# laertispappas/MPI-k-selection

Measured on AMD Instinct MI355X. Metric: Gkeys/s exact k-th select, 2^30 int32 (1 GPU) / 2^33 (8 GPU); % HBM roofline, higher is better.
Workload: dtype int32; 1 GPU; exact k-th select (median) of 2^30 int32 keys per GPU, uniform_half; n_total=1073741824, k=536870912, keys_per_gpu=1073741824, family=uniform_half, parallelism=single, ranks=1

## Files before the change

include/kth.h:

```cpp
#ifndef KTH_H
#define KTH_H

#include <stddef.h>
#include <stdint.h>

#ifdef __cplusplus
extern "C" {
#endif

#define KTH_OK 0
#define KTH_EINVAL (-1)
#define KTH_ENOMEM (-2)
#define KTH_EHIP (-3)
#define KTH_ENODEV (-4)
#define KTH_EINTERNAL (-5)
#define KTH_ECOMM (-6)

#define KTH_VERSION 1

#define KTH_PATH_LDS 1
#define KTH_PATH_RADIX 2
#define KTH_PATH_WINDOW 3
#define KTH_PATH_WINDOW_FALLBACK 4
#define KTH_PATH_K16 5
#define KTH_PATH_K16_FALLBACK 6

typedef struct kth_ctx kth_ctx;

typedef struct kth_stats {
    int32_t path;
    int32_t mode;
    uint32_t lo_key, hi_key;
    uint64_t n, k;
    uint64_t cnt_lt;
    uint64_t cnt_eq_lo, cnt_eq_hi;
    uint64_t candidates;
    uint64_t capacity;
    int32_t answer;
    int32_t error;
} kth_stats;

const char *kth_strerror(int code);
int kth_version(void);
const char *kth_build_id(void);
int kth_device_count(void);

int kth_select_i32(const int32_t *keys, int64_t n, int64_t k, int32_t *out);

int kth_ctx_create(int device, kth_ctx **ctx);
int kth_ctx_destroy(kth_ctx *ctx);
int kth_ctx_set_stream(kth_ctx *ctx, void *hip_stream);
int kth_ctx_sync(kth_ctx *ctx);
int kth_ctx_reserve(kth_ctx *ctx, int64_t n);

int kth_select_i32_ctx(kth_ctx *ctx, const int32_t *keys, int64_t n, int64_t k, int32_t *out);

int kth_select_i32_async(kth_ctx *ctx, const int32_t *d_keys, int64_t n, int64_t k, int32_t *d_out);

int kth_select_f32(const float *keys, int64_t n, int64_t k, float *out);
int kth_select_f32_ctx(kth_ctx *ctx, const float *keys, int64_t n, int64_t k, float *out);
int kth_select_f32_async(kth_ctx *ctx, const float *d_keys, int64_t n, int64_t k, float *d_out);
uint32_t kth_f32_order_key(float x);
float kth_f32_of_order_key(uint32_t key);

#define KTH_MULTI_MAX_RANKS 8
int kth_select_multi_i32(const int32_t *keys, int64_t n, const int64_t *ks, int m, int32_t *out);
int kth_select_multi_i32_ctx(kth_ctx *ctx, const int32_t *keys, int64_t n, const int64_t *ks, int m, int32_t *out);
int kth_select_multi_i32_async(kth_ctx *ctx, const int32_t *d_keys, int64_t n, const int64_t *ks, int m,
                               int32_t *d_out);
int kth_select_multi_f32(const float *keys, int64_t n, const int64_t *ks, int m, float *out);
int kth_select_multi_f32_ctx(kth_ctx *ctx, const float *keys, int64_t n, const int64_t *ks, int m, float *out);
int kth_select_multi_f32_async(kth_ctx *ctx, const float *d_keys, int64_t n, const int64_t *ks, int m, float *d_out);
int kth_ctx_reserve_multi(kth_ctx *ctx, int64_t n, int m);
int kth_ctx_multi_stats(kth_ctx *ctx, int i, kth_stats *st);

#define KTH_K16_I16  0
#define KTH_K16_U16  1
#define KTH_K16_F16  2
#define KTH_K16_BF16 3
uint16_t kth_k16_order_key(uint16_t bits, int kind);
uint16_t kth_k16_of_order_key(uint16_t key, int kind);
int kth_select_k16(const void *keys, int64_t n, int64_t k, int kind, uint16_t *out);
int kth_select_k16_ctx(kth_ctx *ctx, const void *keys, int64_t n, int64_t k, int kind, uint16_t *out);
int kth_select_k16_async(kth_ctx *ctx, const void *d_keys, int64_t n, int64_t k, int kind, uint16_t *d_out);
int kth_select_multi_k16(const void *keys, int64_t n, const int64_t *ks, int m, int kind, uint16_t *out);
int kth_select_multi_k16_ctx(kth_ctx *ctx, const void *keys, int64_t n, const int64_t *ks, int m, int kind,
                             uint16_t *out);
int kth_select_multi_k16_async(kth_ctx *ctx, const void *d_keys, int64_t n, const int64_t *ks, int m, int kind,
                               uint16_t *d_out);
int kth_ctx_reserve_k16(kth_ctx *ctx, int64_t n, int m);

int kth_ctx_last_stats(kth_ctx *ctx, kth_stats *st);

#define KTH_FINISH_NONE 0
#define KTH_FINISH_COUNTS 1
#define KTH_FINISH_SLICES 2
#define KTH_FINISH_GROUPED 3
#define KTH_FINISH_LEVELS 4
int kth_ctx_last_finish_form(kth_ctx *ctx, int *form);

int kth_ctx_coop(const kth_ctx *ctx);

#define KTH_HOOK_FAULT_TOPK_RANK 1
#define KTH_HOOK_FAULT_BARRIER 2
#define KTH_HOOK_TOPK_SEG_CAP 3
#define KTH_HOOK_K16_MISS 4
#define KTH_HOOK_FINISH_SLICES 5
#define KTH_HOOK_K16_TOPK_NOSKIP 6
int kth_ctx_test_hook(kth_ctx *ctx, int hook, int64_t value);

int kth_ctx_enable_timing(kth_ctx *ctx, int on);
int kth_ctx_take_timing(kth_ctx *ctx, int64_t *n_selects, double *main_ms, double *total_ms);

#define KTH_ROWS_MAX_COLS 16384
int kth_select_rows_i32(kth_ctx *ctx, const int32_t *d_keys, int64_t rows, int32_t cols, int32_t k,
                        int32_t *d_out);
int kth_select_rows_f32(kth_ctx *ctx, const float *d_keys, int64_t rows, int32_t cols, int32_t k,
                        float *d_out);

#define KTH_TOPK_MAX_COLS 4096
int kth_topk_rows_i32(kth_ctx *ctx, const int32_t *d_keys, int64_t rows, int32_t cols, int32_t k, int largest,
                      int32_t *d_vals, int32_t *d_idx);
int kth_topk_rows_f32(kth_ctx *ctx, const float *d_keys, int64_t rows, int32_t cols, int32_t k, int largest,
                      float *d_vals, int32_t *d_idx);

#define KTH_ROWS16_MAX_COLS 8192
int kth_select_rows_k16(kth_ctx *ctx, const void *d_keys, int64_t rows, int32_t cols, int32_t k,
                        int kind, uint16_t *d_out);
int kth_topk_rows_k16(kth_ctx *ctx, const void *d_keys, int64_t rows, int32_t cols, int32_t k, int largest,
                      int kind, uint16_t *d_vals, int32_t *d_idx);

int kth_topk_i32(kth_ctx *ctx, const int32_t *d_keys, int64_t n, int64_t k, int largest, int32_t *d_vals,
                 int64_t *d_idx);
int kth_topk_f32(kth_ctx *ctx, const float *d_keys, int64_t n, int64_t k, int largest, float *d_vals,
                 int64_t *d_idx);

int kth_topk_k16(kth_ctx *ctx, const void *d_keys, int64_t n, int64_t k, int largest, int kind,
                 uint16_t *d_vals, int64_t *d_idx);
int kth_ctx_last_topk_k16_tiles(kth_ctx *ctx, uint64_t *tiles, uint64_t *tiles_read);

#define KTH_WIDE_MAX_COLS   (1 << 24)
#define KTH_WIDE_MAX_SLICES 256
int kth_select_wide_rows_i32(kth_ctx *ctx, const int32_t *d_keys, int64_t rows, int32_t cols, int64_t ld, int32_t k,
                             int32_t *d_out);
int kth_select_wide_rows_f32(kth_ctx *ctx, const float *d_keys, int64_t rows, int32_t cols, int64_t ld, int32_t k,
                             float *d_out);
int kth_topk_wide_rows_i32(kth_ctx *ctx, const int32_t *d_keys, int64_t rows, int32_t cols, int64_t ld, int32_t k,
                           int largest, int32_t *d_vals, int32_t *d_idx);
int kth_topk_wide_rows_f32(kth_ctx *ctx, const float *d_keys, int64_t rows, int32_t cols, int64_t ld, int32_t k,
                           int largest, float *d_vals, int32_t *d_idx);
int kth_ctx_reserve_wide_rows(kth_ctx *ctx, int64_t rows, int32_t cols);
int kth_wide_rows_plan(int64_t rows, int32_t cols, int num_cu, int32_t *slices, int32_t *slice_keys,
                       int32_t *group_rows, int64_t *scratch_bytes);
int kth_ctx_wide_rows_force(kth_ctx *ctx, int32_t slices, int32_t group_rows);

int kth_select_wide_rows_k16(kth_ctx *ctx, const void *d_keys, int64_t rows, int32_t cols, int64_t ld,
                             int32_t k, int kind, uint16_t *d_out);
int kth_topk_wide_rows_k16(kth_ctx *ctx, const void *d_keys, int64_t rows, int32_t cols, int64_t ld,
                           int32_t k, int largest, int kind, uint16_t *d_vals, int32_t *d_idx);
int kth_wide_rows_plan_k16(int64_t rows, int32_t cols, int num_cu, int32_t *slices, int32_t *slice_keys,
                           int32_t *group_rows, int64_t *scratch_bytes);

int kth_select_wide_rows_var_i32(kth_ctx *ctx, const int32_t *d_keys, int64_t rows, int32_t cols, int64_t ld,
                                 const int32_t *d_lens, const int32_t *d_ks, int32_t k, int32_t *d_out);
int kth_select_wide_rows_var_f32(kth_ctx *ctx, const float *d_keys, int64_t rows, int32_t cols, int64_t ld,
                                 const int32_t *d_lens, const int32_t *d_ks, int32_t k, float *d_out);
int kth_select_wide_rows_var_k16(kth_ctx *ctx, const void *d_keys, int64_t rows, int32_t cols, int64_t ld,
                                 const int32_t *d_lens, const int32_t *d_ks, int32_t k, int kind, uint16_t *d_out);
int kth_topk_wide_rows_var_i32(kth_ctx *ctx, const int32_t *d_keys, int64_t rows, int32_t cols, int64_t ld,
                               const int32_t *d_lens, const int32_t *d_ks, int32_t k, int largest, int32_t *d_vals,
                               int32_t *d_idx, int32_t *d_cnt);
int kth_topk_wide_rows_var_f32(kth_ctx *ctx, const float *d_keys, int64_t rows, int32_t cols, int64_t ld,
                               const int32_t *d_lens, const int32_t *d_ks, int32_t k, int largest, float *d_vals,
                               int32_t *d_idx, int32_t *d_cnt);
int kth_topk_wide_rows_var_k16(kth_ctx *ctx, const void *d_keys, int64_t rows, int32_t cols, int64_t ld,
                               const int32_t *d_lens, const int32_t *d_ks, int32_t k, int largest, int kind,
                               uint16_t *d_vals, int32_t *d_idx, int32_t *d_cnt);

int kth_fill_synthetic(kth_ctx *ctx, int32_t *d_out, int64_t n, int64_t offset, int64_t n_total,
                       int dist, uint64_t seed, int32_t param);

int kth_nucleus_wide_rows_f32(kth_ctx *ctx, const float *d_keys, int64_t rows, int32_t cols, int64_t ld,
// ... 59 lines not shown
```

mpi-k-selection_amd/csrc/kth_api.hip:

```cpp
#include <hip/hip_runtime.h>

#include <algorithm>
#include <array>
#include <cmath>
#include <cstdio>
#include <cstdlib>
#include <cstring>
#include <vector>

#include "kth.h"
#include "kth_internal.h"
#include "kth_kernels.hip"
#include "kth_topk.hpp"
#include "kth_k16.hpp"
#include "kth_topk16.hpp"

using kth::SelState;
using kth::StepArgs;
using kth::u64;

namespace {

constexpr int64_t SMALL_N = 16384;
constexpr int64_t RADIX_MAX_N = 1ll << 22;
constexpr int64_t SAMPLE_MAX = 1ll << 20;
constexpr double WINDOW_Z = 5.0;
double window_z() {
    static const double z = [] {
        const char *e = getenv("KTH_WINDOW_Z");
        const double v = e ? atof(e) : 0.0;
        return v > 0.0 ? v : WINDOW_Z;
    }();
    return z;
}
constexpr int LEVEL_GRID_MAX = 1024;
constexpr int POST_DENSE_GRID = 256;
constexpr int64_t HEAD_PER_WG = 16 * 1024;
constexpr int HEAD_GRID_MAX = 64;
static_assert(HEAD_GRID_MAX == SAMPLE_MAX / HEAD_PER_WG, "k_head's grid covers the largest sample");
int gather_grid(u64 nchunks) {
    const u64 per_wg = (u64)(kth::DENSE_BLK / kth::WAVE) * kth::GATHER_BATCH;
    return (int)std::max<u64>(1, (nchunks + per_wg - 1) / per_wg);
}
constexpr size_t ISLOT_WORDS = 3 * (size_t)kth::STATS_WORDS + 2;
constexpr size_t HSLOT_OFF = ISLOT_WORDS;
constexpr size_t HSLOT_WORDS = (size_t)kth::HEAD_LEVELS * kth::STATS_WORDS;
constexpr size_t FSLOT_OFF = HSLOT_OFF + HSLOT_WORDS;
constexpr size_t FSLOT_WORDS = (size_t)kth::FIN_LEVELS * kth::STATS_WORDS;
constexpr size_t PRE_OFF = FSLOT_OFF + FSLOT_WORDS;
static_assert(kth::PRE_WORDS % 4 == 0 && PRE_OFF % 2 == 0, "k_finish clears PreHist in 16-byte words");
constexpr size_t ZERO_WORDS = PRE_OFF + (size_t)kth::PRE_WORDS / 2;
constexpr size_t BAR_OFF = ZERO_WORDS;
constexpr size_t TAIL_OFF = BAR_OFF + kth::BAR_WORDS / 2;
constexpr size_t SLOT_ALLOC_WORDS = TAIL_OFF + kth::FIN_LDS_KEYS / 2;
static_assert(kth::BAR_TAIL % 2 == 0, "the tail word is a u64");
constexpr u64 FIN_SPARSE_PER_WG = (u64)kth::DENSE_BLK * kth::FIN_UNROLL * 4;
constexpr double HEAD_SLACK = 1.5;
static_assert(KTH_STATS_WORDS == kth::STATS_WORDS, "include/kth.h slot size");
constexpr int MAX_EVENTS = 4 * 2048;
constexpr u64 TK_STAGE_MAX_FRAC = 16;
constexpr int TK5_SPLIT = 4;
constexpr int COOP_BACKOFF = 64;
constexpr uint64_t DSCAN_PER_WG = 1ull << 16;
constexpr size_t MSET_HSLOT_OFF = ISLOT_WORDS;
constexpr size_t MSET_WORDS = MSET_HSLOT_OFF + HSLOT_WORDS;
static_assert(KTH_MULTI_MAX_RANKS == kth::MULTI_MAX, "include/kth.h rank limit");
constexpr int MULTI_VARIANTS = 3;
constexpr size_t K16_SHIST_WORDS = kth::K16_VALUES / 2;
constexpr size_t K16_BUF_WORDS = K16_SHIST_WORDS + (size_t)KTH_MULTI_MAX_RANKS * kth::K16_RANK_WORDS;
constexpr size_t K16_HIST_LDS = (size_t)kth::K16_VALUES * 2;
static_assert(KTH_K16_I16 == 0 && KTH_K16_U16 == 1 && KTH_K16_F16 == 2 && KTH_K16_BF16 == 3, "kth_k16.hpp's key kinds");
static_assert(KTH_PATH_K16 == 5 && KTH_PATH_K16_FALLBACK == 6, "kth_k16.hpp's paths");

#define HIP_TRY(x)                                                                                    \
    do {                                                                                              \
        hipError_t e_ = (x);                                                                          \
        if (e_ != hipSuccess) {                                                                       \
            if (getenv("KTH_DEBUG")) fprintf(stderr, "kth: %s failed: %s\n", #x, hipGetErrorString(e_)); \
            return KTH_EHIP;                                                                          \
        }                                                                                             \
    } while (0)

#define KTH_TRY(x)              \
    do {                        \
        int r_ = (x);           \
        if (r_ != KTH_OK) return r_; \
    } while (0)

template <typename T>
struct DevBuf {
    T *p = nullptr;
    u64 count = 0;

    int reserve(u64 want) {
        if (count >= want) return KTH_OK;
        (void)hipDeviceSynchronize();
        release();
        if (hipMalloc(reinterpret_cast<void **>(&p), want * sizeof(T)) != hipSuccess) {
            (void)hipGetLastError();
            p = nullptr;
            return KTH_ENOMEM;
        }
        count = want;
        return KTH_OK;
    }
    void release() {
        if (p) (void)hipFree(p);
        p = nullptr;
        count = 0;
    }
};
template <typename... Bufs>
void release_all(Bufs &...bufs) {
    (bufs.release(), ...);
}

}

struct kth_ctx {
    int device = 0;
    int main_grid[2][7] = {};
    int multi_grid[2][MULTI_VARIANTS] = {};
    int main_wg_per_cu = 0;
    bool fault_topk_rank = false;
    bool fault_barrier = false;
    bool fault_once = false;
    bool topk_stage = true;
    u64 topk_seg_cap = 0;
    u64 sparse_per_wg = 0;
    int post_dense_grid = POST_DENSE_GRID;
    int post_sparse_grid = LEVEL_GRID_MAX;
    bool coop = true;
    bool coop_wanted = true;
    int coop_backoff = 0;
    bool coop_resident = true;
    int fin_grid = 256;
    uint32_t head_slack64 = (uint32_t)(HEAD_SLACK * 64);
    uint32_t head_abs_div = 1024;
    bool pre_hist = true;
    bool group = true;
    bool finish_slices = false;
    hipStream_t stream = nullptr;
    bool own_stream = false;
    int num_cu = 256;
    SelState *st = nullptr;
    u64 *islots = nullptr;
    DevBuf<uint32_t> sample;
    DevBuf<uint32_t> cand;
    DevBuf<uint32_t> gdir;
    DevBuf<uint32_t> cand_rows;
    DevBuf<int32_t> tk_segv;
    DevBuf<uint8_t> tk_segp;
    DevBuf<uint32_t> tk_wcnt;
    DevBuf<uint32_t> tk_wstart;
    kth::TkSeg tk_seg{};
    DevBuf<int32_t> staging;
    DevBuf<u64> topk;
    int32_t *d_status = nullptr;
    int32_t *h_status = nullptr;
    SelState *h_state = nullptr;
    int last_state = -1;
    uint32_t multi_tag = 0;
    DevBuf<SelState> mstate;
    DevBuf<u64> mslots;
    DevBuf<uint32_t> mcand;
    int32_t *d_mstatus = nullptr, *h_mstatus = nullptr;
    int multi_m = 0;
    uint32_t multi_word = 0;
    int multi_set[KTH_MULTI_MAX_RANKS] = {};
    u64 multi_cap = 0;
    bool multi_dirty = false;
    DevBuf<u64> k16;
    DevBuf<kth::K16State> k16st;
    int k16_grid[3] = {};
    bool k16_ready = false;
    bool k16_dirty = false;
    bool k16_miss = false;
    int k16_tf_grid[3] = {};
    u64 tk16_tiles = 0;
    DevBuf<u64> tk16_nread;
    bool k16_topk_noskip = false;
    DevBuf<uint32_t> wide_hist;
    DevBuf<kth::WideState> wide_state;
    DevBuf<uint32_t> wide_cnt;
    bool wide_dirty = false;
    int32_t wide_force_slices = 0, wide_force_group = 0;
    DevBuf<u64> tp_mass;
    DevBuf<uint32_t> tp_cnt;
    DevBuf<kth::TpState> tp_state;
    DevBuf<int32_t> tp_rank;
    bool tp_dirty = false;
    DevBuf<kth::SmState> sm_state;
    DevBuf<uint32_t> sm_loc;
    bool sm_dirty = false;
    bool timing = false;
    std::vector<hipEvent_t> ev_main, ev_total;
    int main_used = 0, total_used = 0;
    bool dirty = false;
    bool count_kept = false;
    bool dist_zero = false;
    bool dist_open = false;
    bool dist_coop_window = false;
    bool counts_left = false;
    u64 *stamps = nullptr;
    int stamp_next = 0;
    u64 *uslots = nullptr;
    int64_t dist_n = 0, dist_k = 0, dist_cap = 0;
    int dist_level_next = 0;
    u64 dscan_per_wg = DSCAN_PER_WG;
    int dist_levels = -1;
    int dist_result_slot = -1;
    int32_t *dist_early_out = nullptr;
    uint32_t *h_dist = nullptr;
    uint32_t *d_dist = nullptr;
    hipEvent_t ev_dist = nullptr;
    uint32_t dist_tag = 0;
};

namespace {

u64 *cand_count(kth_ctx *c) { return c->islots + 3 * (size_t)kth::STATS_WORDS; }

enum : uint32_t { LAST_NONE = 0, LAST_SINGLE = 1, LAST_MULTI = 2, LAST_K16 = 3 };
// ... 178 lines not shown
void over_keys(StepArgs &a, const int32_t *keys, int64_t n) {
    a.keys = keys;
    a.n_local = (u64)n;
}
void over_sample(StepArgs &a, const uint32_t *sample, int64_t s) {
    a.sample = sample;
    a.sample_count = (u64)s;
}
void init_rank(StepArgs &a, int64_t n, int64_t k, int64_t s = 0, u64 r_lo = 0, u64 r_hi = 0) {
    a.init_n = (u64)n;
    a.init_k = (u64)k;
    a.init_s = (u64)s;
    a.r_lo = r_lo;
    a.r_hi = r_hi;
}

void ev_mark(kth_ctx *c, std::vector<hipEvent_t> &pool, int &used) {
    if (!c->timing || used >= (int)pool.size()) return;
    (void)hipEventRecord(pool[used++], c->stream);
}
void ev_main(kth_ctx *c) { ev_mark(c, c->ev_main, c->main_used); }

int launch_check() {
    hipError_t e = hipGetLastError();
    if (e != hipSuccess) {
        if (getenv("KTH_DEBUG")) fprintf(stderr, "kth: launch failed: %s\n", hipGetErrorString(e));
        return KTH_EHIP;
    }
    return KTH_OK;
}

constexpr u64 DENSE_PER_WG = 1ull << 16;
constexpr u64 SPARSE_PER_WG = (u64)kth::BLK * kth::LEVEL_UNROLL * 4;

int level_grid(u64 count, u64 per_wg) {
    u64 g = (count + per_wg - 1) / per_wg;
    return (int)std::max<u64>(1, std::min<u64>(LEVEL_GRID_MAX, g));
}

u64 sparse_wg(const kth_ctx *c) { return c->sparse_per_wg ? c->sparse_per_wg : SPARSE_PER_WG; }

template <bool F32 = false>
void launch_level(kth_ctx *c, StepArgs a, bool dense, int grid) {
    if (dense) {
        a.min_per_wg = DENSE_PER_WG;
        kth::k_level<kth::DENSE_BLK, F32><<<grid, kth::DENSE_BLK, 0, c->stream>>>(a);
    } else {
        a.min_per_wg = sparse_wg(c);
        kth::k_level<kth::BLK, F32><<<grid, kth::BLK, 0, c->stream>>>(a);
    }
}

template <bool F32>
int run_small(kth_ctx *c, const int32_t *keys, int64_t n, int64_t k, int32_t *d_out, int32_t *d_status) {
    c->last_state = 1;
    ev_main(c);
    kth::k_small<F32><<<1, kth::SMALL_BLOCK, (size_t)n * 4, c->stream>>>(keys, (u64)n, (u64)k, d_out, d_status,
                                                                    c->st + 1, d_last(c), single_word<F32>(c, 1));
    ev_main(c);
    return launch_check();
}

kth::CoopArgs coop_args(kth_ctx *c, u64 slot_off, int32_t *d_out, int32_t *d_status) {
    kth::CoopArgs x;
    memset(&x, 0, sizeof x);
    x.slots = c->islots + slot_off;
    x.bar = reinterpret_cast<uint32_t *>(c->islots + BAR_OFF);
    x.tail = reinterpret_cast<uint32_t *>(c->islots + TAIL_OFF);
    x.d_out = d_out;
    x.d_status = d_status;
    x.dense_per_wg = DENSE_PER_WG;
    x.sparse_per_wg = FIN_SPARSE_PER_WG;
    x.slack64 = c->head_slack64;
    x.fault = c->fault_barrier ? 1u : 0u;
    if (c->fault_once) c->fault_barrier = false;
    return x;
}

constexpr size_t FIN_DYN_LDS = (size_t)kth::FIN_LDS_KEYS * 4;
uint32_t *pre_words(kth_ctx *c) { return reinterpret_cast<uint32_t *>(c->islots + PRE_OFF); }

template <bool F32>
void launch_finish(kth_ctx *c, const StepArgs &a, int32_t *d_out, int32_t *d_status, uint32_t last, bool with_pre = false,
                   u64 *head_slots = nullptr, int group_rows = 0) {
    kth::CoopArgs x = coop_args(c, FSLOT_OFF, d_out, d_status);
    x.zero2 = head_slots ? head_slots : c->islots + HSLOT_OFF;
    x.zero2_words = HSLOT_WORDS;
    x.pre = with_pre ? pre_words(c) : nullptr;
    x.last = d_last(c);
    kth::FinGroup fg{nullptr, 0u};
    if (with_pre && group_rows > 0 && !c->finish_slices)
        fg = kth::FinGroup{reinterpret_cast<const uint8_t *>(c->gdir.p), (uint32_t)group_rows};
    kth::k_finish<F32><<<c->fin_grid, kth::DENSE_BLK, FIN_DYN_LDS, c->stream>>>(a, x, last, fg);
}

template <bool F32>
int run_radix(kth_ctx *c, const int32_t *keys, int64_t n, int64_t k, int32_t *d_out, int32_t *d_status) {
    if (c->coop) {
        StepArgs a = Chain{c, c->islots, 3}.next(kth::ADV_INIT_FULL, Chain::NONE);
        over_keys(a, keys, n);
        init_rank(a, n, k);
        ev_main(c);
        launch_finish<F32>(c, a, d_out, d_status, single_word<F32>(c, 1));
        ev_main(c);
        c->last_state = 1;
        return launch_check();
    }
    Chain ch{c, c->islots};
    StepArgs a = ch.next(kth::ADV_INIT_FULL, Chain::ACC | Chain::ZERO);
    over_keys(a, keys, n);
    init_rank(a, n, k);
    ev_main(c);
    launch_level<F32>(c, a, true, level_grid((u64)n, DENSE_PER_WG));
    ev_main(c);
    for (int digit = 1; digit <= 2; ++digit) {
        a = ch.next(kth::ADV_PICK);
        over_keys(a, keys, n);
        launch_level<F32>(c, a, false, level_grid((u64)n, sparse_wg(c)));
    }
    a = ch.next(kth::ADV_PICK, Chain::IN);
    kth::k_result<F32><<<1, kth::BLK, 0, c->stream>>>(a, d_out, d_status, c->islots, ISLOT_WORDS, d_last(c),
                                                     single_word<F32>(c, 1));
    c->last_state = 1;
    return launch_check();
}

StepArgs head_step(Chain &ch, int64_t n, int64_t k, int64_t s, u64 r_lo, u64 r_hi, bool clear_counts) {
    StepArgs a = ch.next(kth::ADV_INIT_SAMPLE, clear_counts ? Chain::ZERO : Chain::NONE);
    if (clear_counts) a.zero_words = 2 * (u64)kth::STATS_WORDS + 1;
    init_rank(a, n, k, s, r_lo, r_hi);
    return a;
}

template <bool F32>
void launch_main(kth_ctx *c, const StepArgs &a, int tflag, uint32_t *tflags, uint32_t *gdir = nullptr) {
    const kth::TkSeg none{};
    if (F32 && tflag >= 5) tflag = 0;
    const int g = c->main_grid[F32][tflag];
    uint32_t *cand = c->cand.p, *rows = c->cand_rows.p;
    switch (tflag) {
    case 1: kth::k_main<1, F32><<<g, kth::BLK, 0, c->stream>>>(a, cand, tflags, nullptr, none); break;
    case 2: kth::k_main<2, F32><<<g, kth::BLK, 0, c->stream>>>(a, cand, tflags, nullptr, none); break;
    case 3: kth::k_main<3, F32><<<g, kth::BLK, 0, c->stream>>>(a, cand, tflags, rows, none); break;
    case 4: kth::k_main<4, F32><<<g, kth::BLK, 0, c->stream>>>(a, cand, tflags, rows, none); break;
    case 5:
        if constexpr (!F32) kth::k_main<5><<<g, kth::BLK, 0, c->stream>>>(a, cand, tflags, nullptr, c->tk_seg);
        break;
    case 6:
        if constexpr (!F32) kth::k_main<6><<<g, kth::BLK, 0, c->stream>>>(a, cand, tflags, nullptr, c->tk_seg);
        break;
    default: kth::k_main<0, F32><<<g, kth::BLK, 0, c->stream>>>(a, cand, gdir, nullptr, none); break;
    }
}

template <bool F32>
int run_window(kth_ctx *c, const int32_t *keys, int64_t n, int64_t k, int32_t *d_out, int32_t *d_status,
               int tflag = 0, uint32_t *tflags = nullptr) {
    const int64_t s = sample_size(n);
    const u64 nchunks = ((u64)s + kth::SAMPLE_CHUNK - 1) / kth::SAMPLE_CHUNK;
    const u64 stride = (u64)n / nchunks;
    u64 r_lo, r_hi;
    window_ranks(n, k, s, &r_lo, &r_hi);
    KTH_TRY(reserve_window(c, n));

    if (c->coop) {
        Chain ch{c, c->islots, 2};
        StepArgs a = head_step(ch, n, k, s, r_lo, r_hi, true);
        kth::CoopArgs hx = coop_args(c, HSLOT_OFF, nullptr, nullptr);
        if (tflag == 0 && c->head_abs_div) hx.abs_min = (u64)s / c->head_abs_div;
        kth::k_head<F32><<<gather_grid(nchunks), kth::DENSE_BLK, 0, c->stream>>>(a, hx, keys, (u64)n, stride,
                                                                               c->sample.p, (u64)s);
        a = ch.next(kth::ADV_CARRY, Chain::ACC);
        over_keys(a, keys, n);
        const bool pre = tflag == 0 && c->pre_hist;
        if (pre) a.pre_hist = pre_words(c);
        const bool grp = pre && grouping(c) && c->gdir.p != nullptr;
        ev_main(c);
        launch_main<F32>(c, a, tflag, tflags, grp ? c->gdir.p : nullptr);
        ev_main(c);
        a = ch.next(kth::ADV_DECIDE, Chain::IN);
        over_keys(a, keys, n);
        launch_finish<F32>(c, a, d_out, d_status, single_word<F32>(c, 0), pre, nullptr, grp ? c->main_grid[F32][0] : 0);
        c->last_state = 0;
        c->counts_left = true;
        return launch_check();
    }
    Chain ch{c, c->islots};
    StepArgs a = ch.next(kth::ADV_INIT_SAMPLE, Chain::ACC | Chain::ZERO);
    init_rank(a, n, k, s, r_lo, r_hi);
    kth::k_gather<true, F32><<<gather_grid(nchunks), kth::DENSE_BLK, 0, c->stream>>>(a, keys, (u64)n, stride,
                                                                                   c->sample.p, (u64)s);
    const int gs = level_grid((u64)s, sparse_wg(c));
    for (int digit = 2; digit <= 3; ++digit) {
        a = ch.next(kth::ADV_PICK);
        over_sample(a, c->sample.p, s);
        launch_level(c, a, false, gs);
    }
    a = ch.next(kth::ADV_PICK);
    over_keys(a, keys, n);
    ev_main(c);
    launch_main<F32>(c, a, tflag, tflags);
    ev_main(c);
    a = ch.next(kth::ADV_DECIDE);
    over_keys(a, keys, n);
    launch_level<F32>(c, a, true, c->post_dense_grid);
    for (int digit = 2; digit <= 3; ++digit) {
        a = ch.next(kth::ADV_PICK);
        over_keys(a, keys, n);
        launch_level<F32>(c, a, false, c->post_sparse_grid);
    }
    a = ch.next(kth::ADV_PICK, Chain::IN);
    const bool keep_count = tflag == 3 || tflag == 4;
    kth::k_result<F32><<<1, kth::BLK, 0, c->stream>>>(a, d_out, d_status, c->islots,
                                                     keep_count ? 3 * (u64)kth::STATS_WORDS : (u64)ISLOT_WORDS,
                                                     d_last(c), single_word<F32>(c, 1));
    if (keep_count) c->count_kept = true;
    c->last_state = 1;
    return launch_check();
}

void coop_tick(kth_ctx *c) {
    if (c->coop_backoff > 0 && --c->coop_backoff == 0) c->coop = c->coop_wanted;
}

template <bool F32 = false>
int select_enqueue(kth_ctx *c, const int32_t *d_keys, int64_t n, int64_t k, int32_t *d_out, int32_t *d_status,
                   int tflag = 0, uint32_t *tflags = nullptr) {
    if (c->dirty || c->count_kept) {
        HIP_TRY(hipMemsetAsync(c->islots, 0, SLOT_ALLOC_WORDS * sizeof(u64), c->stream));
        c->dirty = c->count_kept = false;
    }
    int rc;
    ev_mark(c, c->ev_total, c->total_used);
    if (n <= SMALL_N)
        rc = run_small<F32>(c, d_keys, n, k, d_out, d_status);
    else if (n <= RADIX_MAX_N)
        rc = run_radix<F32>(c, d_keys, n, k, d_out, d_status);
    else
        rc = run_window<F32>(c, d_keys, n, k, d_out, d_status, tflag, tflags);
    ev_mark(c, c->ev_total, c->total_used);
    if (rc != KTH_OK) c->dirty = true;
    if (c->stamps) dump_stamps(c);
    return rc;
}

template <bool F32 = false>
int select_async(kth_ctx *c, const int32_t *d_keys, int64_t n, int64_t k, int32_t *d_out, int32_t *d_status,
                 int tflag = 0, uint32_t *tflags = nullptr) {
    if (!c || !d_keys || (!d_out && !d_status) || n < 1 || k < 1 || k > n) return KTH_EINVAL;
    KTH_TRY(set_device(c));
    coop_tick(c);
    return select_enqueue<F32>(c, d_keys, n, k, d_out, d_status, tflag, tflags);
}

bool is_device_ptr(const void *p) {
    hipPointerAttribute_t at;
    hipError_t e = hipPointerGetAttributes(&at, p);
    if (e != hipSuccess) {
        (void)hipGetLastError();
        return false;
    }
    return at.type == hipMemoryTypeDevice || at.type == hipMemoryTypeManaged;
}

thread_local kth_ctx *tl_ctx = nullptr;
// ... 438 lines not shown
        HIP_TRY(hipMemsetAsync(c->sm_state.p, 0, c->sm_state.count * sizeof(kth::SmState), c->stream));
    c->sm_dirty = false;
    return KTH_OK;
}

template <class K, bool VEC>
int launch_sample_group(kth_ctx *c, const WidePlan &p, const typename K::elem *keys, int64_t g, uint32_t cols, u64 ld,
                        const kth::TopP &v, bool no_a, const float *us, int32_t *d_tok, int32_t *d_cnt) {
    if (p.slices == 1) {
        kth::k_sm_fused<K, VEC><<<(int)g, kth::WD_FBLOCK, 0, c->stream>>>(keys, ld, cols, v, us, d_tok, d_cnt);
        return launch_check();
    }
    const dim3 grid((unsigned)p.slices, (unsigned)g);
    const uint32_t sk = (uint32_t)p.slice_keys;
    kth::k_sm_max<K, VEC><<<grid, kth::WD_BLOCK, 0, c->stream>>>(keys, ld, cols, sk, c->sm_state.p, v);
    for (int phase = no_a ? 1 : 0; phase < 2; ++phase)
        for (int pass = 0; pass < K::PASSES; ++pass) {
            kth::k_sm_count<K, VEC><<<grid, kth::WD_BLOCK, 0, c->stream>>>(keys, ld, cols, sk, phase, pass, c->tp_mass.p,
                                                                        c->tp_cnt.p, c->sm_state.p, v);
            kth::k_sm_pick<K><<<(int)g, kth::WD_BLOCK, 0, c->stream>>>(c->tp_mass.p, c->tp_cnt.p, c->sm_state.p, phase, pass,
                                                                     cols, v, us);
        }
    kth::k_sm_loc_count<K, VEC><<<grid, kth::WD_BLOCK, 0, c->stream>>>(keys, ld, cols, sk, c->sm_state.p, c->sm_loc.p, v);
    kth::k_sm_loc_pick<K, VEC><<<grid, kth::WD_BLOCK, 0, c->stream>>>(keys, ld, cols, sk, c->sm_state.p, c->sm_loc.p, v,
                                                                   d_tok, d_cnt);
    const int rc = launch_check();
    if (rc != KTH_OK) c->tp_dirty = c->sm_dirty = true;
    return rc;
}

template <class K>
int sample_rows(kth_ctx *c, const typename K::elem *keys, int64_t rows, int32_t cols, int64_t ld, const kth::TopP &var,
                bool no_a, const float *d_us, int32_t *d_tok, int32_t *d_cnt) {
    constexpr int32_t align = K::PER;
    WidePlan p = wide_plan(rows, cols, c->num_cu, c->wide_force_slices, c->wide_force_group, align,
                           align == 8 ? WIDE16_MIN_SLICE : WIDE_MIN_SLICE);
    if (p.slices > 1) {
        p.group_rows = (int32_t)std::min<int64_t>(p.group_rows, SM_GROUP_MAX);
        KTH_TRY(reserve_sample(c, p.group_rows));
    }
    const bool vec = (reinterpret_cast<uintptr_t>(keys) & 15u) == 0 && ld % align == 0;
    const auto launch = vec ? launch_sample_group<K, true> : launch_sample_group<K, false>;
    for (int64_t r0 = 0; r0 < rows; r0 += p.group_rows) {
        const int64_t g = std::min<int64_t>(p.group_rows, rows - r0);
        kth::TopP v = var;
        if (v.lens) v.lens += r0;
        if (v.ps) v.ps += r0;
        if (v.temps) v.temps += r0;
        if (v.ks) v.ks += r0;
        KTH_TRY(launch(c, p, keys + (u64)r0 * (u64)ld, g, (uint32_t)cols, (u64)ld, v, no_a, d_us + r0, d_tok + r0,
                       d_cnt ? d_cnt + r0 : nullptr));
    }
    return KTH_OK;
}

int sample_entry(kth_ctx *c, const void *d_keys, int64_t rows, int32_t cols, int64_t ld, const int32_t *d_lens,
                 const int32_t *d_ks, int32_t k, const float *d_ps, float p, const float *d_temps, float temp,
                 const float *d_us, int kind, int32_t *d_tok, int32_t *d_cnt) {
    if (!c || !d_keys || !d_us || !d_tok || rows < 0 || cols < 1 || cols > KTH_WIDE_MAX_COLS || ld < cols)
        return KTH_EINVAL;
    if (kind != -1 && kind != KTH_K16_F16 && kind != KTH_K16_BF16) return KTH_EINVAL;
    if (!(temp > 0.0f) || !std::isfinite(temp) || (!d_ps && std::isnan(p))) return KTH_EINVAL;
    if (rows == 0) return KTH_OK;
    KTH_TRY(set_device(c));
    const kth::TopP var{d_lens, d_ps, d_temps, d_ks, p, temp, k};
    const bool no_a = !d_ps && p >= 1.0f && !d_ks && k <= 0;
    if (kind == -1)
        return sample_rows<kth::TpF32>(c, static_cast<const uint32_t *>(d_keys), rows, cols, ld, var, no_a, d_us, d_tok,
                                       d_cnt);
    const uint16_t *keys = static_cast<const uint16_t *>(d_keys);
    if (kind == KTH_K16_BF16) return sample_rows<kth::TpK16<true>>(c, keys, rows, cols, ld, var, no_a, d_us, d_tok, d_cnt);
    return sample_rows<kth::TpK16<false>>(c, keys, rows, cols, ld, var, no_a, d_us, d_tok, d_cnt);
}

void read_tuning(kth_ctx *c) {
    if (const char *g = getenv("KTH_MAIN_WG_PER_CU")) c->main_wg_per_cu = std::max(0, atoi(g));
    if (const char *g = getenv("KTH_SPARSE_PER_WG")) c->sparse_per_wg = (u64)std::max(0, atoi(g));
    if (const char *g = getenv("KTH_DSCAN_PER_WG")) c->dscan_per_wg = (u64)std::max(1024, atoi(g));
    if (const char *g = getenv("KTH_POST_DENSE_GRID")) c->post_dense_grid = std::max(1, atoi(g));
    if (const char *g = getenv("KTH_POST_SPARSE_GRID")) c->post_sparse_grid = std::max(1, atoi(g));
    if (const char *g = getenv("KTH_COOP")) c->coop = atoi(g) != 0;
    if (const char *g = getenv("KTH_PRE_HIST")) c->pre_hist = atoi(g) != 0;
    if (const char *g = getenv("KTH_GROUP")) c->group = atoi(g) != 0;
    c->fin_grid = c->num_cu;
    if (const char *g = getenv("KTH_FIN_GRID")) c->fin_grid = std::max(1, std::min(atoi(g), c->num_cu));
    if (const char *g = getenv("KTH_HEAD_SLACK")) c->head_slack64 = (uint32_t)std::max(0.0, atof(g) * 64.0);
    if (const char *g = getenv("KTH_HEAD_ABS")) c->head_abs_div = (uint32_t)std::max(0, atoi(g));
    if (const char *g = getenv("KTH_TOPK_STAGE")) c->topk_stage = atoi(g) != 0;
}

template <int TF, bool F32>
const void *main_fn() {
    if constexpr (F32 && TF >= 5)
        return nullptr;
    else
        return reinterpret_cast<const void *>(kth::k_main<TF, F32>);
}
template <bool F32>
std::array<const void *, 7> main_fns() {
    return {main_fn<0, F32>(), main_fn<1, F32>(), main_fn<2, F32>(), main_fn<3, F32>(),
            main_fn<4, F32>(), main_fn<5, F32>(), main_fn<6, F32>()};
}

template <bool F32>
std::array<const void *, 7 + MULTI_VARIANTS> pass_fns() {
    const std::array<const void *, 7> f = main_fns<F32>();
    return {f[0], f[1], f[2], f[3], f[4], f[5], f[6],
            reinterpret_cast<const void *>(kth::k_main_multi<2, F32>),
            reinterpret_cast<const void *>(kth::k_main_multi<4, F32>),
            reinterpret_cast<const void *>(kth::k_main_multi<8, F32>)};
}
int pass_grid(const kth_ctx *c, const void *fn) {
    int per = 4;
    hipFuncAttributes fa;
    if (hipFuncGetAttributes(&fa, fn) == hipSuccess && fa.numRegs > 0) {
        const int alloc = (fa.numRegs + 7) / 8 * 8;
        const int by_vgpr = std::min(8, 512 / alloc);
        const int lds = (int)fa.sharedSizeBytes;
        const int by_lds = lds > 0 ? (160 * 1024) / lds : 8;
        per = std::max(1, std::min(by_vgpr, by_lds));
    }
    (void)hipGetLastError();
    if (c->main_wg_per_cu > 0) per = c->main_wg_per_cu;
    return c->num_cu * per;
}
void size_main_grids(kth_ctx *c) {
    const std::array<const void *, 7 + MULTI_VARIANTS> fns[2] = {pass_fns<false>(), pass_fns<true>()};
    for (int kind = 0; kind < 2; ++kind)
        for (int tf = 0; tf < 7 + MULTI_VARIANTS; ++tf) {
            if (!fns[kind][tf]) continue;
            (tf < 7 ? c->main_grid[kind][tf] : c->multi_grid[kind][tf - 7]) = pass_grid(c, fns[kind][tf]);
        }
}

template <bool F32>
bool coop_per_cu(int *fin, int *head) {
    return hipOccupancyMaxActiveBlocksPerMultiprocessor(fin, reinterpret_cast<const void *>(kth::k_finish<F32>),
                                                        kth::DENSE_BLK, FIN_DYN_LDS) == hipSuccess &&
           hipOccupancyMaxActiveBlocksPerMultiprocessor(head, reinterpret_cast<const void *>(kth::k_head<F32>),
                                                        kth::DENSE_BLK, 0) == hipSuccess;
}

bool coop_grids_resident(const kth_ctx *c) {
    int fin[2] = {0, 0}, head[2] = {0, 0};
    const bool known = coop_per_cu<false>(&fin[0], &head[0]) && coop_per_cu<true>(&fin[1], &head[1]);
    (void)hipGetLastError();
    if (!known) return true;
    return (int64_t)std::min(fin[0], fin[1]) * c->num_cu >= c->fin_grid &&
           (int64_t)std::min(head[0], head[1]) * c->num_cu >= HEAD_GRID_MAX;
}

}

extern "C" {

const char *kth_strerror(int code) {
    switch (code) {
    case KTH_OK: return "ok";
    case KTH_EINVAL: return "invalid argument";
    case KTH_ENOMEM: return "out of memory";
    case KTH_EHIP: return "HIP runtime error";
    case KTH_ENODEV: return "no HIP device";
    case KTH_EINTERNAL: return "device-side consistency check failed";
    case KTH_ECOMM: return "RCCL unavailable or a collective failed";
    default: return "unknown error";
    }
// ... 681 lines not shown
    return KTH_OK;
}

int fetch_stats(kth_ctx *c, const SelState *d_state, u64 capacity, bool f32, kth_stats *out) {
    KTH_TRY(set_device(c));
    HIP_TRY(hipMemcpyAsync(c->h_state, d_state, sizeof(SelState), hipMemcpyDeviceToHost, c->stream));
    HIP_TRY(hipStreamSynchronize(c->stream));
    const SelState &s = *c->h_state;
    memset(out, 0, sizeof *out);
    out->path = (int32_t)s.path;
    out->mode = (int32_t)s.mode;
    out->lo_key = s.lo;
    out->hi_key = s.hi;
    out->n = s.n;
    out->k = s.k;
    out->cnt_lt = s.cnt[kth::C_LT];
    out->cnt_eq_lo = s.cnt[kth::C_EQLO];
    out->cnt_eq_hi = s.cnt[kth::C_EQHI];
    out->candidates = s.cnt[kth::C_IN];
    out->capacity = capacity;
    out->answer = f32 ? (int32_t)kth::f32_of_key(s.answer) : (int32_t)(s.answer ^ 0x80000000u);
    out->error = (int32_t)s.error;
    return KTH_OK;
}

int fetch_stats_k16(kth_ctx *c, int j, int kind, kth_stats *out) {
    KTH_TRY(set_device(c));
    kth::K16State *h = reinterpret_cast<kth::K16State *>(c->h_state);
    static_assert(sizeof(kth::K16State) <= sizeof(SelState), "the pinned state buffer holds either");
    HIP_TRY(hipMemcpyAsync(h, c->k16st.p + j, sizeof *h, hipMemcpyDeviceToHost, c->stream));
    HIP_TRY(hipStreamSynchronize(c->stream));
    memset(out, 0, sizeof *out);
    out->path = (int32_t)h->path;
    out->mode = (int32_t)h->mode;
    out->lo_key = kth::k16_key_of_ord(h->lo, kind);
    out->hi_key = kth::k16_key_of_ord(h->hi, kind);
    out->n = h->n;
    out->k = h->k;
    out->cnt_lt = h->cnt_lt;
    out->candidates = h->inside;
    out->answer = (int32_t)kth::k16_bits_of_ord(h->answer, kind);
    out->error = (int32_t)h->error;
    return KTH_OK;
}

int last_stats(kth_ctx *c, const LastCall &last, kth_stats *out) {
    switch (last.form) {
    case LAST_K16: return fetch_stats_k16(c, last.index, last.k16_kind, out);
    case LAST_MULTI: return fetch_stats(c, c->mstate.p + 2 * (size_t)last.index, c->multi_cap, last.f32, out);
    case LAST_SINGLE: return fetch_stats(c, c->st + (last.index & 1), c->cand.count, last.f32, out);
    default: return KTH_EINVAL;
    }
}

int multi_stats(kth_ctx *c, int i, kth_stats *out) {
    if (!c || !out || i < 0 || i >= c->multi_m) return KTH_EINVAL;
    LastCall last;
    KTH_TRY(fetch_last(c, &last));
    const LastCall mine = last_of_word(c->multi_word);
    if (last.form != mine.form || last.f32 != mine.f32 || last.k16_kind != mine.k16_kind) return KTH_EINVAL;
    last.index = c->multi_set[i];
    return last_stats(c, last, out);
}

}

extern "C" {

int kth_ctx_multi_stats(kth_ctx *c, int i, kth_stats *out) { return multi_stats(c, i, out); }

int kth_ctx_last_stats(kth_ctx *c, kth_stats *out) {
    if (!c || !out) return KTH_EINVAL;
    LastCall last;
    KTH_TRY(fetch_last(c, &last));
    return last_stats(c, last, out);
}

int kth_ctx_last_finish_form(kth_ctx *c, int *form) {
    if (!c || !form) return KTH_EINVAL;
    LastCall last;
    KTH_TRY(fetch_last(c, &last));
    if (last.form == LAST_NONE) return KTH_EINVAL;
    *form = (int)((uint32_t)c->h_status[2] >> kth::LAST_FORM_SHIFT & 7u);
    return KTH_OK;
}

int kth_ctx_enable_timing(kth_ctx *c, int on) {
    if (!c) return KTH_EINVAL;
    KTH_TRY(set_device(c));
    if (on && c->ev_main.empty()) {
        c->ev_main.resize(MAX_EVENTS);
        c->ev_total.resize(MAX_EVENTS);
        for (auto &e : c->ev_main) HIP_TRY(hipEventCreate(&e));
        for (auto &e : c->ev_total) HIP_TRY(hipEventCreate(&e));
    }
    c->timing = on != 0;
    c->main_used = c->total_used = 0;
    return KTH_OK;
}

int kth_ctx_take_timing(kth_ctx *c, int64_t *n_sel, double *main_ms, double *total_ms) {
    if (!c || !n_sel || !main_ms || !total_ms) return KTH_EINVAL;
    KTH_TRY(set_device(c));
    HIP_TRY(hipStreamSynchronize(c->stream));
    double m = 0, t = 0;
    int64_t nm = 0;
    for (int i = 0; i + 1 < c->main_used; i += 2) {
        float a = 0;
        HIP_TRY(hipEventElapsedTime(&a, c->ev_main[i], c->ev_main[i + 1]));
        m += a;
        nm++;
    }
    for (int i = 0; i + 1 < c->total_used; i += 2) {
        float b = 0;
        HIP_TRY(hipEventElapsedTime(&b, c->ev_total[i], c->ev_total[i + 1]));
        t += b;
    }
    c->main_used = c->total_used = 0;
    *n_sel = nm;
    *main_ms = m;
    *total_ms = t;
    return KTH_OK;
}

int kth_select_rows_i32(kth_ctx *c, const int32_t *d_keys, int64_t rows, int32_t cols, int32_t k, int32_t *d_out) {
    return rows_entry<false, false>(c, d_keys, rows, cols, k, d_out);
}

int kth_select_rows_f32(kth_ctx *c, const float *d_keys, int64_t rows, int32_t cols, int32_t k, float *d_out) {
    return rows_entry<true, false>(c, d_keys, rows, cols, k, d_out);
}

int kth_topk_rows_i32(kth_ctx *c, const int32_t *d_keys, int64_t rows, int32_t cols, int32_t k, int largest,
                      int32_t *d_vals, int32_t *d_idx) {
    return rows_entry<false, true>(c, d_keys, rows, cols, k, nullptr, largest, d_vals, d_idx);
}

int kth_topk_rows_f32(kth_ctx *c, const float *d_keys, int64_t rows, int32_t cols, int32_t k, int largest,
                      float *d_vals, int32_t *d_idx) {
    return rows_entry<true, true>(c, d_keys, rows, cols, k, nullptr, largest, d_vals, d_idx);
}

int kth_select_rows_k16(kth_ctx *c, const void *d_keys, int64_t rows, int32_t cols, int32_t k, int kind,
                        uint16_t *d_out) {
    return rows16_entry<false>(c, d_keys, rows, cols, k, kind, d_out);
}

int kth_topk_rows_k16(kth_ctx *c, const void *d_keys, int64_t rows, int32_t cols, int32_t k, int largest, int kind,
                      uint16_t *d_vals, int32_t *d_idx) {
    return rows16_entry<true>(c, d_keys, rows, cols, k, kind, nullptr, largest, d_vals, d_idx);
}

int kth_select_wide_rows_i32(kth_ctx *c, const int32_t *d_keys, int64_t rows, int32_t cols, int64_t ld, int32_t k,
                             int32_t *d_out) {
    return wide_rows_entry<false, false>(c, d_keys, rows, cols, ld, k, d_out);
}

int kth_select_wide_rows_f32(kth_ctx *c, const float *d_keys, int64_t rows, int32_t cols, int64_t ld, int32_t k,
                             float *d_out) {
    return wide_rows_entry<true, false>(c, d_keys, rows, cols, ld, k, d_out);
}

int kth_topk_wide_rows_i32(kth_ctx *c, const int32_t *d_keys, int64_t rows, int32_t cols, int64_t ld, int32_t k,
                           int largest, int32_t *d_vals, int32_t *d_idx) {
    return wide_rows_entry<false, true>(c, d_keys, rows, cols, ld, k, nullptr, largest, d_vals, d_idx);
}
// ... 615 lines not shown
```

mpi-k-selection_amd/csrc/kth_coop.hpp:

```cpp
#pragma once

namespace kth {

struct CoopArgs {
    u64 *slots;
    uint32_t *bar;
    int32_t *d_out, *d_status;
    u64 dense_per_wg, sparse_per_wg;
    uint32_t slack64;
    u64 abs_min;
    u64 *zero2;
    u64 zero2_words;
    uint32_t *tail;
    uint32_t sample_ready;
    uint32_t fault;
    uint32_t *pre;
    uint32_t *last;
};

template <int BLOCK>
__device__ __forceinline__ void pick_slot_copies(SelState &ss, const u64 *slot, uint32_t nb, uint32_t copies,
                                                 u64 *tmp , u64 *scratch, u64 *cnt0) {
    constexpr int PER = NBINS / BLOCK;
#pragma unroll
// ... 58 lines not shown
    __shared__ SelState ss;
    __shared__ u64 scratch[2 * (DENSE_BLK / WAVE) + 8];
    __shared__ __attribute__((aligned(16))) uint32_t lh[2][NBINS];
    __shared__ uint32_t s_base[BAR_NG];
    KTH_STAMP(a, 0);
    GridBar gb = grid_bar_init(x.bar, s_base);
    for (int i = threadIdx.x; i < 2 * NBINS / 4; i += DENSE_BLK) reinterpret_cast<uint4 *>(&lh[0][0])[i] = make_uint4(0, 0, 0, 0);
    for (u64 i = (u64)blockIdx.x * DENSE_BLK + threadIdx.x; i < a.zero_words; i += (u64)gridDim.x * DENSE_BLK)
        a.stats_zero[i] = 0;
    advance<DENSE_BLK>(ss, a, scratch);
    bool share;
    HistPlan plan = make_plan(ss, &share);
    auto hist_sample = [&]() {
        const CoherentBuf sb(sample, (uint32_t)(s * 4));
        const uint32_t nv = (uint32_t)(s / 4), per = DENSE_BLK * HEAD_UNROLL;
        for (uint32_t v0 = blockIdx.x * per; v0 < nv; v0 += gridDim.x * per) {
            uint4 q[HEAD_UNROLL];
#pragma unroll
            for (int u = 0; u < HEAD_UNROLL; ++u) {
                const uint32_t v = v0 + u * DENSE_BLK + threadIdx.x;
                q[u] = sb.load16(v < nv ? v * 16u : 0u);
            }
#pragma unroll
            for (int u = 0; u < HEAD_UNROLL; ++u) {
                const bool in = v0 + u * DENSE_BLK + threadIdx.x < nv;
                hist_add<DENSE_BLK>(lh, plan, q[u].x, in);
                hist_add<DENSE_BLK>(lh, plan, q[u].y, in);
                hist_add<DENSE_BLK>(lh, plan, q[u].z, in);
                hist_add<DENSE_BLK>(lh, plan, q[u].w, in);
            }
        }
    };
    bool from_chunks = false;
    if (x.sample_ready)
        hist_sample();
    else if (gather_head_fast<DENSE_BLK, F32>(keys, stride, s, lh, plan, blockIdx.x, gridDim.x))
        from_chunks = true;
    else
        gather_chunks<DENSE_BLK, true, true, F32>(keys, n_keys, stride, sample, s, lh, plan);
    hist_flush<DENSE_BLK>(lh, plan, x.slots);
    KTH_STAMP(a, 1);
    const EarlyWindow ew{a.r_lo, a.r_hi, x.slack64, x.abs_min};
    bool ok = true;
    for (int L = 0;; ++L) {
        grid_sync(gb, s_base, ok);
        if (x.fault) ok = false;
        if (L == 0) KTH_STAMP(a, 2);
        if (L == 1) KTH_STAMP(a, 5);
        pick_slot<DENSE_BLK>(ss, x.slots + (size_t)L * STATS_WORDS, share, scratch, &ew);
        if (L == 0) KTH_STAMP(a, 3);
        if (L == 1) KTH_STAMP(a, 6);
        if (ss.mode != MODE_SAMPLE || L + 1 >= HEAD_LEVELS) break;
        plan = make_plan(ss, &share);
        for (int i = threadIdx.x; i < 2 * NBINS / 4; i += DENSE_BLK)
            reinterpret_cast<uint4 *>(&lh[0][0])[i] = make_uint4(0, 0, 0, 0);
        __syncthreads();
        if (from_chunks)
            head_hist_chunks<DENSE_BLK, F32>(keys, stride, s, lh, plan, blockIdx.x, gridDim.x);
        else
            hist_sample();
        hist_flush<DENSE_BLK>(lh, plan, x.slots + (size_t)(L + 1) * STATS_WORDS);
        if (L == 0) KTH_STAMP(a, 4);
    }
    if (blockIdx.x == 0 && threadIdx.x == 0) {
        SelState o = ss;
        const uint32_t berr = __hip_atomic_exchange(x.bar + BAR_ERR, 0u, __ATOMIC_RELAXED, __HIP_MEMORY_SCOPE_AGENT);
        if ((!ok || berr) && !o.error) {
            o.error = ERR_BARRIER;
            o.mode = MODE_DONE;
        } else if (o.mode == MODE_SAMPLE && !o.error) {
            o.error = 16 + o.mode;
            o.mode = MODE_DONE;
        }
        o.share = 0;
        *a.st_out = o;
    }
    grid_bar_finish(gb, s_base);
    KTH_STAMP(a, 7);
}

constexpr int FIN_LDS_KEYS = 32768;
constexpr int FIN_UNROLL = 4;
constexpr uint32_t LAST_FORM_SHIFT = 12;

__device__ __forceinline__ void finish_keys(uint32_t (*lh)[NBINS], const HistPlan &plan, const uint4 &x, bool xr,
                                            uint32_t valid4) {
    const uint32_t X = xr ? 0x80000000u : 0u;
    hist_add<DENSE_BLK>(lh, plan, x.x ^ X, valid4 & 1u);
    hist_add<DENSE_BLK>(lh, plan, x.y ^ X, valid4 & 2u);
    hist_add<DENSE_BLK>(lh, plan, x.z ^ X, valid4 & 4u);
    hist_add<DENSE_BLK>(lh, plan, x.w ^ X, valid4 & 8u);
}

constexpr uint32_t TAIL_STAGE = 2 * NBINS;

__device__ __forceinline__ uint32_t finisher_pad(const SelState &ss) {
    return ss.base + ((ss.t[0].prefix ^ 1u) << (ss.W - ss.t[0].done));
}

template <bool F32>
__device__ __forceinline__ void finish_levels(const StepArgs &a, SelState &ss, const uint4 *res, uint32_t total,
                                              uint32_t (*lh)[NBINS], u64 *scratch) {
    __shared__ uint32_t s_ln;
    __shared__ uint32_t s_list[WAVE];
    __shared__ u64 s_c;
    const uint32_t W = ss.W, base = ss.base, nq = (total + 3) / 4, pad = finisher_pad(ss);
    const int lane = threadIdx.x & (WAVE - 1);
    constexpr int PER = NBINS / DENSE_BLK;
    for (int it = 0; ss.mode == MODE_CAND || ss.mode == MODE_FULL; ++it) {
        (void)it;
        const uint32_t dn = ss.t[0].done, pf = ss.t[0].prefix, d = digit_bits(ss, dn);
        const uint32_t msh = W - dn, sh = W - dn - d, mask = (1u << d) - 1u;
        for (int i = threadIdx.x; i < NBINS / 4; i += DENSE_BLK) reinterpret_cast<uint4 *>(&lh[0][0])[i] = make_uint4(0, 0, 0, 0);
        __syncthreads();
        auto add = [&](uint32_t key) {
            const uint32_t v = key - base;
            if ((v >> msh) == pf) atomicAdd(&lh[0][(v >> sh) & mask], 1u);
        };
        for (uint32_t v = threadIdx.x; v < nq; v += DENSE_BLK) {
            const uint4 q = res[v];
            add(q.x);
            add(q.y);
            add(q.z);
            add(q.w);
        }
        __syncthreads();
        u64 h0[PER];
#pragma unroll
        for (int j = 0; j < PER; ++j) h0[j] = lh[0][threadIdx.x * PER + j];
        pick_state<DENSE_BLK, PER>(ss, h0, h0, true, scratch, nullptr, &s_c);
#ifdef KTH_STAMPS_BUILD
        if (it < 2) KTH_STAMP(a, 1 + it);
#endif
        if ((ss.mode == MODE_CAND || ss.mode == MODE_FULL) && s_c <= (u64)WAVE) {
            const uint32_t dl = ss.t[0].done, pl = ss.t[0].prefix, msl = W - dl;
            if (threadIdx.x == 0) s_ln = 0;
            __syncthreads();
            auto put = [&](uint32_t key) {
                const bool m = ((key - base) >> msl) == pl;
                const u64 b = __ballot(m);
                if (b == 0) return;
                uint32_t at = 0;
                if (lane == 0) at = atomicAdd(&s_ln, (uint32_t)__popcll(b));
                at = __shfl(at, 0, WAVE);
                const uint32_t i = at + (uint32_t)__builtin_amdgcn_mbcnt_hi((uint32_t)(b >> 32),
                                                                             __builtin_amdgcn_mbcnt_lo((uint32_t)b, 0u));
                if (m && i < (uint32_t)WAVE) s_list[i] = key;
            };
            for (uint32_t v0 = 0; v0 < nq; v0 += DENSE_BLK) {
                const uint32_t v = v0 + threadIdx.x;
                const uint4 q = v < nq ? res[v] : make_uint4(pad, pad, pad, pad);
                put(q.x);
                put(q.y);
                put(q.z);
                put(q.w);
            }
            __syncthreads();
            if (threadIdx.x < WAVE) {
                const uint32_t ln = s_ln < (uint32_t)WAVE ? s_ln : (uint32_t)WAVE;
                const uint32_t mine = (uint32_t)lane < ln ? s_list[lane] : 0u;
                uint32_t lt = 0, le = 0;
                for (uint32_t j = 0; j < ln; ++j) {
                    const uint32_t o = s_list[j];
                    lt += o < mine ? 1u : 0u;
                    le += o <= mine ? 1u : 0u;
                }
// ... 73 lines not shown
            const uint32_t valid4 = nk - e >= 4 ? 0xFu : (1u << (uint32_t)(nk - e)) - 1u;
            const uint32_t k4[4] = {q.x ^ X, q.y ^ X, q.z ^ X, q.w ^ X};
#pragma unroll
            for (int j = 0; j < 4; ++j)
                if (((valid4 >> j) & 1u) && ((k4[j] - base) >> psh) == prefix) {
                    const uint32_t i = atomicAdd(&s_pos, 1u);
                    if (off + i < (uint32_t)FIN_LDS_KEYS)
                        __hip_atomic_store(x.tail + off + i, k4[j], __ATOMIC_RELAXED, __HIP_MEMORY_SCOPE_AGENT);
                }
        }
    }
    wait_mem();
    __syncthreads();
    uint32_t *written = x.bar + BAR_TAIL_WRITTEN;
    if (!s_last) {
        if (threadIdx.x == 0) __hip_atomic_fetch_add(written, 1u, __ATOMIC_RELAXED, __HIP_MEMORY_SCOPE_AGENT);
        KTH_STAMP(a, 5);
        return false;
    }
    if (threadIdx.x == 0) {
        uint32_t spins = 0;
        while (__hip_atomic_load(written, __ATOMIC_RELAXED, __HIP_MEMORY_SCOPE_AGENT) != gridDim.x - 1u) {
            __builtin_amdgcn_s_sleep(1);
            if (++spins >= BAR_SPIN_LIMIT) {
                ss.error = ERR_BARRIER;
                ss.mode = MODE_DONE;
                break;
            }
        }
        __hip_atomic_store(written, 0u, __ATOMIC_RELAXED, __HIP_MEMORY_SCOPE_AGENT);
        __hip_atomic_store(ctl, 0ull, __ATOMIC_RELAXED, __HIP_MEMORY_SCOPE_AGENT);
        if (x.fault) {
            ss.error = ERR_BARRIER;
            ss.mode = MODE_DONE;
        }
    }
    __syncthreads();
    KTH_STAMP(a, 5);
    if (ss.error) return true;
    const uint32_t total = s_total;
    if (total > (uint32_t)FIN_LDS_KEYS) {
        if (threadIdx.x == 0) {
            ss.error = 32;
            ss.mode = MODE_DONE;
        }
        __syncthreads();
        return true;
    }
    const uint32_t nq = (total + 3) / 4;
    const uint32_t pad = base + ((prefix ^ 1u) << psh);
    {
        constexpr int TU = FIN_LDS_KEYS / 4 / DENSE_BLK;
        static_assert(TU % FIN_UNROLL == 0, "tail loads in FIN_UNROLL batches");
        const CoherentBuf tb(x.tail, FIN_LDS_KEYS * 4);
        for (int u0 = 0; u0 < TU; u0 += FIN_UNROLL) {
            if ((uint32_t)(u0 * DENSE_BLK) >= nq) break;
            uint4 q[FIN_UNROLL];
#pragma unroll
            for (int u = 0; u < FIN_UNROLL; ++u) {
                const uint32_t v = (u0 + u) * DENSE_BLK + threadIdx.x;
                q[u] = v < nq ? tb.load16(v * 16u) : make_uint4(0, 0, 0, 0);
            }
#pragma unroll
            for (int u = 0; u < FIN_UNROLL; ++u) {
                const uint32_t v = (u0 + u) * DENSE_BLK + threadIdx.x;
                if (v == total / 4 && (total & 3u)) {
                    if ((total & 3u) <= 1) q[u].y = pad;
                    if ((total & 3u) <= 2) q[u].z = pad;
                    q[u].w = pad;
                }
                res[(u0 + u) * DENSE_BLK + threadIdx.x] = q[u];
            }
        }
        __syncthreads();
    }
    KTH_STAMP(a, 6);
    *total_out = total;
    return true;
}

struct FinGroup {
    const uint8_t *dir;
    uint32_t rows;
};
constexpr int GATHER_UNROLL = 8;
template <bool F32>
__device__ bool finish_gather(const StepArgs &a, SelState &ss, const FinGroup &fg, uint4 *res, u64 cnt0,
                              uint32_t (*lh)[NBINS], u64 *scratch, uint32_t *total_out) {
    static_assert(2 * NBINS * 4 >= DENSE_BLK * 12, "the places and sources fit the histogram's LDS");
    uint32_t *off = &lh[0][0];
    u64 *src = reinterpret_cast<u64 *>(&lh[1][0]);
    const uint32_t b = ss.t[0].prefix, pad = finisher_pad(ss);
    uint32_t cnt = 0;
    u64 s0 = 0;
    if (threadIdx.x < fg.rows) {
        const uint8_t *row = fg.dir + (size_t)threadIdx.x * GDIR_ROW_BYTES;
        const uint16_t *P = reinterpret_cast<const uint16_t *>(row);
        const uint32_t p0 = P[b], p1 = P[b + 1];
        s0 = *reinterpret_cast<const u64 *>(row + GDIR_BASE_OFF) + p0;
        cnt = p1 >= p0 ? p1 - p0 : 0u;
    }
    u64 total;
    off[threadIdx.x] = (uint32_t)block_exclusive_scan<DENSE_BLK>((u64)cnt, scratch, &total);
    src[threadIdx.x] = s0;
    __syncthreads();
    KTH_STAMP(a, 5);
    if (total != cnt0 || total > (u64)FIN_LDS_KEYS) {
        if (threadIdx.x == 0) {
            ss.error = 34;
            ss.mode = MODE_DONE;
        }
        __syncthreads();
        return false;
    }
    const uint32_t tot = (uint32_t)total;
    uint32_t *rw = reinterpret_cast<uint32_t *>(res);
    for (uint32_t i0 = 0; i0 < tot; i0 += GATHER_UNROLL * DENSE_BLK) {
        uint32_t v[GATHER_UNROLL];
#pragma unroll
        for (int u = 0; u < GATHER_UNROLL; ++u) {
            const uint32_t i = i0 + u * DENSE_BLK + threadIdx.x;
            v[u] = pad;
            if (i < tot) {
                uint32_t s = 0;
#pragma unroll
                for (uint32_t step = DENSE_BLK / 2; step; step >>= 1) s += off[s + step] <= i ? step : 0u;
                const u64 at = src[s] + (i - off[s]);
                if (at < a.cap) v[u] = load_nt(a.cand + at);
            }
        }
#pragma unroll
        for (int u = 0; u < GATHER_UNROLL; ++u) {
            const uint32_t i = i0 + u * DENSE_BLK + threadIdx.x;
            if (i < tot) rw[i] = v[u];
        }
    }
    if (threadIdx.x < 3 && tot + threadIdx.x < ((tot + 3) & ~3u)) rw[tot + threadIdx.x] = pad;
    __syncthreads();
    KTH_STAMP(a, 6);
    *total_out = tot;
    return true;
}

template <bool F32 = false>
__global__ __launch_bounds__(DENSE_BLK) void k_finish(StepArgs a, CoopArgs x, uint32_t last_tag, FinGroup fg) {
    __shared__ SelState ss;
    __shared__ u64 scratch[2 * (DENSE_BLK / WAVE) + 8];
    __shared__ __attribute__((aligned(16))) uint32_t lh[2][NBINS];
    extern __shared__ uint4 res[];
    __shared__ uint32_t s_base[BAR_NG];
    __shared__ u64 s_cnt0, s_ptot;
    KTH_STAMP(a, 0);
    if (threadIdx.x == 0) s_ptot = 0;
    GridBar gb = grid_bar_init(x.bar, s_base);
    for (int i = threadIdx.x; i < 2 * NBINS / 4; i += DENSE_BLK) reinterpret_cast<uint4 *>(&lh[0][0])[i] = make_uint4(0, 0, 0, 0);
    const uint32_t pre_incomplete = x.pre ? x.pre[PRE_INCOMPLETE] : 1u;
    [[clang::always_inline]] advance<DENSE_BLK>(ss, a, scratch);
    if (threadIdx.x == 0 && (ss.mode == MODE_CAND || ss.mode == MODE_FULL) && ss.t[0].done == 0)
        ss.d0 = fin_first_digit(ss.W);
    __syncthreads();
    const bool use_pre = pre_incomplete == 0u && ss.mode == MODE_CAND && ss.t[0].done == 0;
    const bool group = use_pre && fg.dir != nullptr && fg.rows <= (uint32_t)DENSE_BLK && !x.fault;
    KTH_STAMP(a, 1);
    const uint32_t mode0 = ss.mode;
    const bool live = mode0 == MODE_CAND || mode0 == MODE_FULL;
    const uint32_t *dom = mode0 == MODE_FULL ? reinterpret_cast<const uint32_t *>(a.keys) : a.cand;
    const u64 count = mode0 == MODE_CAND ? min(*a.cand_count, a.cap) : a.n_local;
    const bool xr = mode0 == MODE_FULL;
    const bool aligned = (reinterpret_cast<uintptr_t>(dom) & 15u) == 0;
    const bool resident = live && count <= (u64)gridDim.x * FIN_LDS_KEYS;
    u64 b0 = 0, nk = 0;
    if (resident) {
        const u64 per = ((count + gridDim.x - 1) / gridDim.x + 3) & ~(u64)3;
        b0 = min((u64)blockIdx.x * per, count);
        nk = min(per, count - b0);
    }
    bool ok = true, tail = false, gather = false;
    int levels = 0;
    for (int L = 0; L < FIN_LEVELS; ++L) {
        const uint32_t mode = ss.mode;
        if (mode != MODE_CAND && mode != MODE_FULL) break;
        levels = L + 1;
        bool share;
        const HistPlan plan = make_plan(ss, &share);
        if (L > 0) {
            for (int i = threadIdx.x; i < 2 * NBINS / 4; i += DENSE_BLK)
                reinterpret_cast<uint4 *>(&lh[0][0])[i] = make_uint4(0, 0, 0, 0);
            __syncthreads();
        }
        const bool pre0 = L == 0 && use_pre;
        const uint32_t nb = plan.mask[0] + 1u, copies = L == 0 ? NBINS / nb : 1u;
        if (pre0 && group) {
            pick_pre<DENSE_BLK>(ss, x.pre, nb, scratch, &s_cnt0, &s_ptot);
            if (s_ptot != ss.cnt[C_IN] ||
                ((ss.mode == MODE_CAND || ss.mode == MODE_FULL) && s_cnt0 <= (u64)FIN_LDS_KEYS)) {
                gather = true;
                KTH_STAMP(a, 4);
                break;
            }
        }
        if (resident) {
            const uint32_t nv = (uint32_t)((nk + 3) / 4);
            if (L == 0) {
                const bool one = plan.h[0] && !plan.h[1] && plan.done[0] == 0;
                const uint32_t X = xr ? 0x80000000u : 0u, bs = plan.base, sh = plan.shift[0], mk = plan.mask[0];
                auto add4 = [&](const uint4 &q) {
                    atomicAdd(&lh[0][(((q.x ^ X) - bs) >> sh) & mk], 1u);
                    atomicAdd(&lh[0][(((q.y ^ X) - bs) >> sh) & mk], 1u);
                    atomicAdd(&lh[0][(((q.z ^ X) - bs) >> sh) & mk], 1u);
                    atomicAdd(&lh[0][(((q.w ^ X) - bs) >> sh) & mk], 1u);
                };
                if (aligned) {
                    const uint4 *src = reinterpret_cast<const uint4 *>(dom + b0);
                    for (uint32_t v0 = 0; v0 < nv; v0 += FIN_UNROLL * DENSE_BLK) {
                        uint4 q[FIN_UNROLL];
#pragma unroll
                        for (int u = 0; u < FIN_UNROLL; ++u) {
                            const uint32_t v = v0 + u * DENSE_BLK + threadIdx.x;
                            q[u] = v < nv ? load_nt(src + v) : make_uint4(0, 0, 0, 0);
                        }
#pragma unroll
                        for (int u = 0; u < FIN_UNROLL; ++u) {
                            const uint32_t v = v0 + u * DENSE_BLK + threadIdx.x;
                            if (v < nv) {
                                const u64 e = 4ull * v;
                                if constexpr (F32)
                                    if (xr) q[u] = ord_word4<true>(q[u]);
                                res[v] = q[u];
                                if (pre0)
                                    ;
                                else if (one && nk - e >= 4)
                                    add4(q[u]);
                                else
                                    finish_keys(lh, plan, q[u], xr, nk - e >= 4 ? 0xFu : (1u << (uint32_t)(nk - e)) - 1u);
                            }
                        }
                    }
                } else {
                    for (uint32_t v = threadIdx.x; v < nv; v += DENSE_BLK) {
                        uint4 q = make_uint4(0, 0, 0, 0);
                        const u64 e = b0 + 4ull * v, left = b0 + nk - e;
                        q.x = dom[e];
                        if (left > 1) q.y = dom[e + 1];
                        if (left > 2) q.z = dom[e + 2];
                        if (left > 3) q.w = dom[e + 3];
                        if constexpr (F32)
                            if (xr) q = ord_word4<true>(q);
                        res[v] = q;
                        if (!pre0) finish_keys(lh, plan, q, xr, left >= 4 ? 0xFu : (1u << (uint32_t)left) - 1u);
                    }
                }
            } else {
                for (uint32_t v = threadIdx.x; v < nv; v += DENSE_BLK) {
                    const u64 e = 4ull * v;
                    finish_keys(lh, plan, res[v], xr, nk - e >= 4 ? 0xFu : (1u << (uint32_t)(nk - e)) - 1u);
                }
            }
        } else if (!pre0) {
            const uint32_t active = active_wgs(count, L == 0 ? x.dense_per_wg : x.sparse_per_wg);
            auto f = [&](const uint32_t *k, uint32_t valid, auto full) {
#pragma unroll
                for (int j = 0; j < 4 * FIN_UNROLL; ++j)
                    hist_add<DENSE_BLK>(lh, plan, k[j], decltype(full)::value || ((valid >> j) & 1u));
            };
            if (blockIdx.x < active) {
                if (xr)
                    stream_tiles<DENSE_BLK, FIN_UNROLL, F32 ? 2 : 1>(dom, count, blockIdx.x, active, f);
                else
                    stream_tiles<DENSE_BLK, FIN_UNROLL, 0>(dom, count, blockIdx.x, active, f);
            }
        }
#ifdef KTH_STAMPS_BUILD
        if (pre0) {
            wait_mem();
            KTH_STAMP(a, 2);
        }
#endif
        u64 *slot = x.slots + (size_t)L * STATS_WORDS;
        if (pre0) {
            if (!group) pick_pre<DENSE_BLK>(ss, x.pre, nb, scratch, &s_cnt0);
        } else {
            if (copies > 1)
                hist_flush_copies<DENSE_BLK>(lh, nb, copies, slot);
            else
                hist_flush<DENSE_BLK>(lh, plan, slot);
            if (L == 0) KTH_STAMP(a, 2);
            grid_sync(gb, s_base, ok);
            if (x.fault) ok = false;
            if (L == 0) KTH_STAMP(a, 3);
            if (copies > 1)
                pick_slot_copies<DENSE_BLK>(ss, slot, nb, copies, reinterpret_cast<u64 *>(&lh[0][0]), scratch, &s_cnt0);
            else
                pick_slot<DENSE_BLK>(ss, slot, share, scratch, nullptr, &s_cnt0);
        }
        KTH_STAMP(a, 4 + L);
        if (resident && (ss.mode == MODE_CAND || ss.mode == MODE_FULL) && s_cnt0 <= (u64)FIN_LDS_KEYS) {
            tail = true;
            break;
        }
    }
    const u64 spread = (u64)blockIdx.x * DENSE_BLK + threadIdx.x, step = (u64)gridDim.x * DENSE_BLK;
    if (gather) {
        for (u64 i = spread; i < x.zero2_words; i += step) x.zero2[i] = 0;
        if (blockIdx.x != 0) {
            KTH_STAMP(a, 7);
            return;
        }
    }
    if (levels > 0 && !tail && !gather) grid_sync(gb, s_base, ok);
    grid_bar_finish(gb, s_base);
    bool writer = blockIdx.x == 0, finisher = false;
    uint32_t fin_keys = 0;
    if (tail) {
        [[clang::always_inline]] writer = finisher = finish_tail<F32>(a, ss, x, res, nk, xr, lh, scratch, &fin_keys);
    } else if (gather && (ss.mode == MODE_CAND || ss.mode == MODE_FULL)) {
        [[clang::always_inline]] finisher = finish_gather<F32>(a, ss, fg, res, s_cnt0, lh, scratch, &fin_keys);
    }
    if (finisher && !ss.error) finish_levels<F32>(a, ss, res, fin_keys, lh, scratch);
    const uint32_t form = levels == 0 ? 1u : tail ? 2u : gather ? 3u : 4u;
    if (writer && threadIdx.x == 0) {
        SelState o = ss;
        const uint32_t berr = __hip_atomic_exchange(x.bar + BAR_ERR, 0u, __ATOMIC_RELAXED, __HIP_MEMORY_SCOPE_AGENT);
        if ((!ok || berr) && !o.error) o.error = ERR_BARRIER;
        if (o.mode != MODE_DONE && !o.error) o.error = 16 + o.mode;
        *a.st_out = o;
        if (x.d_out && !o.error) *x.d_out = out_word<F32>(o.answer);
        if (x.d_status) {
            x.d_status[0] = i32_of_key(o.answer);
            x.d_status[1] = (int32_t)o.error;
        }
        if (x.last) *x.last = last_tag | form << LAST_FORM_SHIFT;
    }
    if (gather) {
        for (uint32_t i = threadIdx.x; i < (uint32_t)PRE_WORDS / 4; i += DENSE_BLK)
            reinterpret_cast<uint4 *>(x.pre)[i] = make_uint4(0, 0, 0, 0);
        KTH_STAMP(a, 7);
        return;
    }
    const u64 shared_words = (u64)(tail ? levels - 1 : levels) * STATS_WORDS;
    for (u64 i = spread; i < shared_words; i += step) x.slots[i] = 0;
    for (u64 i = spread; i < x.zero2_words; i += step) x.zero2[i] = 0;
    if (tail) {
        if (writer) {
            if (!(levels == 1 && use_pre))
                for (uint32_t i = threadIdx.x; i < (uint32_t)STATS_WORDS; i += DENSE_BLK) x.slots[shared_words + i] = 0;
            if (x.pre)
                for (uint32_t i = threadIdx.x; i < (uint32_t)PRE_WORDS / 4; i += DENSE_BLK)
                    reinterpret_cast<uint4 *>(x.pre)[i] = make_uint4(0, 0, 0, 0);
        }
    } else if (x.pre) {
        for (u64 i = spread; i < (u64)PRE_WORDS; i += step) x.pre[i] = 0u;
    }
    KTH_STAMP(a, 7);
}

}
```

mpi-k-selection_amd/csrc/kth_gridbar.hpp:

```cpp
#pragma once
#include "kth_device.hpp"

namespace kth {

constexpr int HEAD_LEVELS = 3;
constexpr int FIN_LEVELS = 3;
constexpr int HEAD_UNROLL = 4;
constexpr int BAR_GROUP_STRIDE = 64;
constexpr int BAR_NG = 64;
constexpr int BAR_BASE = BAR_NG * BAR_GROUP_STRIDE;
constexpr int BAR_ERR = BAR_BASE + BAR_GROUP_STRIDE;
constexpr int BAR_TAIL = BAR_ERR + BAR_GROUP_STRIDE;
constexpr int BAR_TAIL_WRITTEN = BAR_TAIL + 32;
constexpr int BAR_TOPK_ARRIVE = BAR_TAIL + 48;
constexpr int BAR_WORDS = BAR_TAIL + BAR_GROUP_STRIDE;
static_assert(BAR_TAIL_WRITTEN >= BAR_TAIL + 2 && BAR_TOPK_ARRIVE > BAR_TAIL_WRITTEN && BAR_TOPK_ARRIVE < BAR_WORDS,
              "the tail word (u64), its written count and the top-k arrival counter are distinct words");
static_assert(BAR_NG <= WAVE && BAR_NG <= BAR_GROUP_STRIDE, "one wave polls every group; the bases fit one stride");
constexpr uint32_t BAR_SPIN_LIMIT = 1u << 21;
constexpr uint32_t ERR_BARRIER = 64;

__device__ __forceinline__ void wait_mem() { asm volatile("s_waitcnt vmcnt(0)" ::: "memory"); }

struct GridBar {
    uint32_t *bar;
    uint32_t n;
};

__device__ __forceinline__ uint32_t group_size(uint32_t g) { return (gridDim.x - g + BAR_NG - 1u) / BAR_NG; }

__device__ __forceinline__ GridBar grid_bar_init(uint32_t *bar, uint32_t *s_base) {
    if (threadIdx.x < BAR_NG) s_base[threadIdx.x] = bar[BAR_BASE + threadIdx.x];
    return GridBar{bar, 0u};
}

__device__ __forceinline__ void grid_sync(GridBar &gb, const uint32_t *s_base, bool &ok) {
    __shared__ uint32_t s_ok;
    wait_mem();
    __syncthreads();
    gb.n++;
    if (threadIdx.x < WAVE) {
        const uint32_t lane = threadIdx.x, groups = gridDim.x < (uint32_t)BAR_NG ? gridDim.x : (uint32_t)BAR_NG;
        if (lane == 0)
            __hip_atomic_fetch_add(gb.bar + (blockIdx.x % BAR_NG) * BAR_GROUP_STRIDE, 1u, __ATOMIC_RELAXED,
                                   __HIP_MEMORY_SCOPE_AGENT);
        const uint32_t target = lane < groups ? s_base[lane] + gb.n * group_size(lane) : 0u;
        bool done = lane >= groups;
        uint32_t spins = 0, good = 1;
        while (true) {
            if (!done) {
                const uint32_t v = __hip_atomic_load(gb.bar + lane * BAR_GROUP_STRIDE, __ATOMIC_RELAXED,
                                                     __HIP_MEMORY_SCOPE_AGENT);
                done = (int32_t)(v - target) >= 0;
            }
            if (__ballot(!done) == 0) break;
            __builtin_amdgcn_s_sleep(1);
            if (++spins >= BAR_SPIN_LIMIT) {
                good = 0;
                if (lane == 0) __hip_atomic_fetch_or(gb.bar + BAR_ERR, 1u, __ATOMIC_RELAXED, __HIP_MEMORY_SCOPE_AGENT);
                break;
            }
        }
        if (lane == 0) s_ok = good;
    }
    __syncthreads();
    ok = ok && s_ok != 0;
}

__device__ __forceinline__ void grid_bar_finish(const GridBar &gb, const uint32_t *s_base) {
    if (blockIdx.x == 0 && threadIdx.x < BAR_NG)
        gb.bar[BAR_BASE + threadIdx.x] = s_base[threadIdx.x] + gb.n * group_size(threadIdx.x);
}

struct CoherentBuf {
    __amdgpu_buffer_rsrc_t r;
    __device__ CoherentBuf(const void *p, uint32_t bytes)
        : r(__builtin_amdgcn_make_buffer_rsrc(const_cast<void *>(p), (short)0, (int)bytes, 0x00020000)) {}
    __device__ __forceinline__ uint4 load16(uint32_t byte_off) const {
        const auto v = __builtin_amdgcn_raw_buffer_load_b128(r, (int)byte_off, 0, 16 );
        return make_uint4(v[0], v[1], v[2], v[3]);
    }
};

}
```

mpi-k-selection_amd/csrc/kth_kernels.hip:

```cpp
#include <type_traits>

#include "kth_device.hpp"
#include "kth_gridbar.hpp"

namespace kth {

constexpr int BLK = 256;
#ifndef KTH_MAIN_UNROLL
#define KTH_MAIN_UNROLL 8
#endif
constexpr int MAIN_UNROLL = KTH_MAIN_UNROLL;
constexpr int MAIN_SUB = MAIN_UNROLL < 8 ? MAIN_UNROLL : 8;
#ifndef KTH_WREG
#define KTH_WREG 2048
#endif
constexpr int WREG = KTH_WREG;
#ifndef KTH_WREG5
#define KTH_WREG5 2496
#endif
constexpr int WREG5 = KTH_WREG5;
constexpr int LEVEL_UNROLL = 8;
constexpr int DENSE_BLK = 1024;
#ifndef KTH_SAMPLE_CK
#define KTH_SAMPLE_CK 16
// ... 791 lines not shown
    __device__ __forceinline__ uint32_t row(const uint4 &q, uint32_t lane, uint32_t &ceqlo, uint32_t &ceqhi) {
        auto f1 = [&](uint32_t x) { return TF == 5 ? (int32_t)x <= shi : (int32_t)x >= slo; };
        const bool c0 = f1(q.x), c1 = f1(q.y), c2 = f1(q.z), c3 = f1(q.w);
        const unsigned long long b0 = __builtin_amdgcn_ballot_w64(c0), b1 = __builtin_amdgcn_ballot_w64(c1),
                                 b2 = __builtin_amdgcn_ballot_w64(c2), b3 = __builtin_amdgcn_ballot_w64(c3);
        if ((b0 | b1 | b2 | b3) == 0) return 0u;
        {
            const int32_t x0 = (int32_t)q.x, x1 = (int32_t)q.y, x2 = (int32_t)q.z, x3 = (int32_t)q.w;
            ceqlo += ((c0 & (x0 == slo)) ? 1u : 0u) + ((c1 & (x1 == slo)) ? 1u : 0u) +
                     ((c2 & (x2 == slo)) ? 1u : 0u) + ((c3 & (x3 == slo)) ? 1u : 0u);
            ceqhi += ((c0 & (x0 == shi)) ? 1u : 0u) + ((c1 & (x1 == shi)) ? 1u : 0u) +
                     ((c2 & (x2 == shi)) ? 1u : 0u) + ((c3 & (x3 == shi)) ? 1u : 0u);
        }
        const uint32_t n0 = (uint32_t)__popcll(b0), n1 = (uint32_t)__popcll(b1), n2 = (uint32_t)__popcll(b2);
        const uint32_t total = n0 + n1 + n2 + (uint32_t)__popcll(b3);
        if (wfill + total > CAP) flush();
        uint8_t *pb = reinterpret_cast<uint8_t *>(reg + CAP);
        auto at = [](unsigned long long b, uint32_t base) {
            return __builtin_amdgcn_mbcnt_hi((uint32_t)(b >> 32), __builtin_amdgcn_mbcnt_lo((uint32_t)b, base));
        };
        const uint32_t a0 = at(b0, wfill), a1 = at(b1, wfill + n0), a2 = at(b2, wfill + n0 + n1),
                       a3 = at(b3, wfill + n0 + n1 + n2);
        if (c0) { reg[a0] = q.x; pb[a0] = (uint8_t)lane; }
        if (c1) { reg[a1] = q.y; pb[a1] = (uint8_t)(WAVE + lane); }
        if (c2) { reg[a2] = q.z; pb[a2] = (uint8_t)(2 * WAVE + lane); }
        if (c3) { reg[a3] = q.w; pb[a3] = (uint8_t)(3 * WAVE + lane); }
        wfill += total;
        return total;
    }
};
static_assert(OrdStager::CAP + OrdStager::CAP / 4 <= (uint32_t)WREG5 && OrdStager::CAP >= 4 * WAVE && WREG <= WREG5,
              "OrdStager region: keys + position bytes in one wave's region, >= one wave-row");

template <int CTRL, int ROWS = 0xF>
__device__ __forceinline__ uint32_t dpp_add(uint32_t x) {
    return (uint32_t)__builtin_amdgcn_update_dpp(0, (int)x, CTRL, ROWS, 0xF, false);
}

struct RowAcc {
    uint32_t r[8];
};

template <int K, bool FULL, bool ROWS, int RW = 0>
__device__ __forceinline__ void scan_keys(const uint32_t (&xw)[K], uint32_t valid, int32_t slo, int32_t shi,
                                          uint32_t &clt, uint32_t &ceqlo, uint32_t &ceqhi, Stager<ROWS> &st,
                                          uint32_t row0 = ~0u, RowAcc *ra = nullptr) {
    static_assert(RW == 0 || (FULL && K == 32), "row tallies cover a full tile's 8 rows");
    const uint32_t span = (uint32_t)shi - (uint32_t)slo;
#pragma unroll
    for (int j = 0; j < K; ++j) {
        const int32_t x = (int32_t)xw[j];
        const bool ok = FULL || ((valid >> j) & 1u);
        clt += (ok & (x < slo)) ? 1u : 0u;
        if constexpr (RW == 3) {
            if ((j & 3) == 3) ra->r[j / 4] = clt;
        } else if constexpr (RW == 4) {
            ra->r[j / 4] += x > shi ? 1u : 0u;
        }
        st.slot_near(x, ok & (xw[j] - (uint32_t)slo <= span), slo, shi, ceqlo, ceqhi,
                     row0 == ~0u ? ~0u : row0 + (uint32_t)(j / 4));
    }
}

constexpr uint32_t TK_RECOUNT = 1u << 31;
constexpr u64 TF_W0 = 64;
constexpr int RW_REGS = 16;
struct RowWords {
    u64 G;
    u64 seg;
};
__host__ __device__ __forceinline__ u64 rw_seg_words(u64 nfull, u64 G) {
    return ((nfull + G - 1) / G * MAIN_UNROLL + 63) / 64 * 64;
}
__host__ __device__ __forceinline__ u64 fl_seg_bytes(u64 nfull, u64 G) { return ((nfull + G - 1) / G + 255) / 256 * 256; }
__host__ __device__ __forceinline__ u64 fl_index(const RowWords &L, u64 t, uint32_t w) {
    return ((t % L.G) * (BLK / WAVE) + w) * L.seg + t / L.G;
}
__host__ __device__ __forceinline__ u64 rw_index(const RowWords &L, u64 r, uint32_t w) {
    const u64 t = r / MAIN_UNROLL;
    return TF_W0 + ((t % L.G) * (BLK / WAVE) + w) * L.seg + (t / L.G) * MAIN_UNROLL + r % MAIN_UNROLL;
}
static_assert(MAIN_UNROLL <= 8, "k_main<TF> keeps one row bit per 16-B load slot in a byte");
static_assert(BLK / WAVE == 4, "k_main<TF> stores one flag byte per wave, four per tile (tk_row_flagged's mask)");
template <int TF, bool F32 = false>
__global__ __launch_bounds__(BLK) void k_main(StepArgs a, uint32_t *__restrict__ cand_out,
                                              uint32_t *__restrict__ tflags, uint32_t *__restrict__ cand_rows,
                                              TkSeg seg) {
    constexpr int U = MAIN_UNROLL, S = MAIN_SUB, K = 4 * S;
    constexpr bool ROWS = TF == 3 || TF == 4;
    constexpr bool ORD = TF >= 5;
    static_assert(!(F32 && ORD), "the staged top-k is int32 only: its segments hold the caller's words");
    static_assert(U % S == 0, "MAIN_UNROLL is a multiple of MAIN_SUB");
    __shared__ SelState ss;
    __shared__ u64 scratch[2 * (BLK / WAVE) + 8];
    __shared__ __attribute__((aligned(16))) uint32_t region[BLK / WAVE][TF >= 5 ? WREG5 : WREG];
    __shared__ u64 red[6][BLK / WAVE];
    __shared__ uint32_t rowx[BLK / WAVE][4];
    KTH_STAMP(a, 0);
    const uint32_t *p = reinterpret_cast<const uint32_t *>(a.keys);
    const u64 n = a.n_local;
    u64 head = ((16u - (uint32_t)(reinterpret_cast<uintptr_t>(p) & 15u)) & 15u) >> 2;
    if (head > n) head = n;
    const uint4 *__restrict__ v = reinterpret_cast<const uint4 *>(p + head);
    const u64 nv = (n - head) >> 2, tail0 = head + (nv << 2);
    const u64 tile = (u64)BLK * U, nfull = nv / tile;
    auto load_tile = [&](uint4 (&x)[U], u64 t) {
        const uint4 *src = v + t * tile + threadIdx.x;
        x[0] = load_nt(src);
        asm volatile("s_waitcnt vmcnt(0)" ::: "memory");
#pragma unroll
        for (int u = 1; u < U; ++u) x[u] = load_nt(src + u * BLK);
    };
    advance<BLK>(ss, a, scratch);
    publish<BLK>(ss, 0, a);
    KTH_STAMP(a, 1);
    if (ss.mode != MODE_MAIN) return;
    const int32_t slo = i32_of_key(ss.lo), shi = i32_of_key(ss.hi);
    const int lane = threadIdx.x & (WAVE - 1), wid = threadIdx.x / WAVE;
    if constexpr (TF != 0) {
        if (blockIdx.x == 0 && threadIdx.x == 0) {
            tflags[0] = (uint32_t)slo;
            tflags[1] = (uint32_t)shi;
            tflags[2] = 1u;
        }
    }
    Stager<ROWS> st{region[wid], 0u, 0ull, a.cand_count, a.stats_acc, a.cap, cand_out, cand_rows, 0u};
    OrdStager os{region[wid], 0u, 0u, 0ull, ((u64)blockIdx.x * (BLK / WAVE) + wid) * seg.cap, slo, shi,
                 a.cand_count, a.stats_acc, a.cap, cand_out, seg};
    uint32_t clt = 0, ceqlo = 0, ceqhi = 0;
    auto ord_keys = [&](const uint4 &q) -> uint32_t {
        clt += ((int32_t)q.x < slo ? 1u : 0u) + ((int32_t)q.y < slo ? 1u : 0u) + ((int32_t)q.z < slo ? 1u : 0u) +
               ((int32_t)q.w < slo ? 1u : 0u);
        return os.template row<TF>(q, (uint32_t)lane, ceqlo, ceqhi);
    };
    auto load_tile_ord = [&](uint4 (&x)[U], u64 t) {
        const uint32_t *src = reinterpret_cast<const uint32_t *>(v + t * tile) + wid * (4 * WAVE) + lane;
        x[0].x = load_nt(src);
        asm volatile("s_waitcnt vmcnt(0)" ::: "memory");
        x[0].y = load_nt(src + WAVE);
        x[0].z = load_nt(src + 2 * WAVE);
        x[0].w = load_nt(src + 3 * WAVE);
#pragma unroll
        for (int u = 1; u < U; ++u) {
            const uint32_t *r = src + u * (4 * BLK);
            x[u] = make_uint4(load_nt(r), load_nt(r + WAVE), load_nt(r + 2 * WAVE), load_nt(r + 3 * WAVE));
        }
    };

    constexpr int RW = (TF == 3 || TF == 4) ? TF : 0;
    auto scan_tile = [&](const uint4 (&x)[U], u64 t, RowAcc &ra) {
        static_assert(RW == 0 || U == S, "row tallies: one key group per tile");
#pragma unroll
        for (int h = 0; h < U / S; ++h) {
            uint32_t kk[K];
#pragma unroll
            for (int u = 0; u < S; ++u) {
                kk[4 * u + 0] = x[h * S + u].x;
                kk[4 * u + 1] = x[h * S + u].y;
                kk[4 * u + 2] = x[h * S + u].z;
                kk[4 * u + 3] = x[h * S + u].w;
            }
            scan_keys<K, true, ROWS, RW>(kk, 0xFFFFFFFFu, slo, shi, clt, ceqlo, ceqhi, st,
                                         ROWS ? (uint32_t)(t * U + h * S) : ~0u, &ra);
        }
    };
    uint32_t tiles_done = 0;
    uint32_t tile_word = 0, grp[RW_REGS], wsr = 0, facc = 0;
    uint32_t *const fseg = TF == 1 || TF == 2
                               ? tflags + 4 + ((u64)blockIdx.x * (BLK / WAVE) + wid) * (fl_seg_bytes(nfull, gridDim.x) / 4)
                               : nullptr;
#pragma unroll
    for (int q = 0; q < RW_REGS; ++q) grp[q] = 0u;
    const u64 seg_words = rw_seg_words(nfull, gridDim.x);
    uint32_t *const wseg = tflags + TF_W0 + ((u64)blockIdx.x * (BLK / WAVE) + wid) * seg_words;
    auto flag_tile = [&](const uint4 (&x)[U], u64 t, RowAcc &ra, uint32_t e0, uint32_t c0) {
        if constexpr (TF == 1 || TF == 2) {
            uint32_t rows = 0;
#pragma unroll
            for (int u = 0; u < U; ++u) {
                const int32_t a0 = (int32_t)x[u].x, a1 = (int32_t)x[u].y, a2 = (int32_t)x[u].z, a3 = (int32_t)x[u].w;
                const bool nr = TF == 1 ? min(min(a0, a1), min(a2, a3)) <= shi : max(max(a0, a1), max(a2, a3)) >= slo;
                rows |= (__builtin_amdgcn_ballot_w64(nr) != 0 ? 1u : 0u) << u;
            }
            facc = (uint32_t)lane == (tiles_done / 4) % WAVE ? facc | rows << (8 * (tiles_done % 4)) : facc;
        }
        if constexpr (TF >= 3) {
            static_assert(U == 8, "k_main<3/4> packs four rows' counts into each of two words");
            if constexpr (TF == 3) {
#pragma unroll
                for (int u = U - 1; u > 0; --u) ra.r[u] -= ra.r[u - 1];
                ra.r[0] -= c0;
            }
            uint32_t b0 = ra.r[0] | ra.r[1] << 8 | ra.r[2] << 16 | ra.r[3] << 24;
            uint32_t b1 = ra.r[4] | ra.r[5] << 8 | ra.r[6] << 16 | ra.r[7] << 24;
            auto half_scan = [](uint32_t c) {
                c += dpp_add<0x111>(c);
                c += dpp_add<0x112>(c);
                c += dpp_add<0x114>(c);
                c += dpp_add<0x118>(c);
                c += dpp_add<0x142, 0xA>(c);
                return c;
// ... 74 lines not shown
    }
    if constexpr (TF >= 3) {
        const uint32_t g0 = tiles_done - tiles_done % (RW_REGS * TK5_WIN_TILES);
#pragma unroll
        for (int q = 0; q < RW_REGS; ++q) {
            const uint32_t t0 = g0 + (uint32_t)q * TK5_WIN_TILES;
            if (t0 < tiles_done && (uint32_t)lane < (tiles_done - t0 < TK5_WIN_TILES ? tiles_done - t0 : TK5_WIN_TILES) * U)
                wseg[t0 * U + lane] = grp[q];
        }
        if constexpr (ORD) {
            const uint32_t wl = tiles_done / TK5_WIN_TILES, w0 = wl - wl % WAVE;
            if (wl % WAVE != WAVE - 1 && (uint32_t)lane <= wl % WAVE && w0 + lane < seg.nwin)
                seg.wstart[((u64)blockIdx.x * (BLK / WAVE) + wid) * seg.nwin + w0 + lane] = wsr;
        }
    }
    if constexpr (ORD) os.flush(true);
    const u64 rem0 = nfull * tile;
    if (blockIdx.x == (uint32_t)(nfull % gridDim.x))
        for (int h = 0; h < U / S; ++h) {
            uint32_t kk[K];
            uint32_t ok = 0;
#pragma unroll
            for (int u = 0; u < S; ++u) {
                const u64 i = rem0 + (h * S + u) * BLK + threadIdx.x;
                const bool in = i < nv;
                const uint4 x = ord_word4<F32>(in ? v[i] : make_uint4(0, 0, 0, 0));
                kk[4 * u + 0] = x.x;
                kk[4 * u + 1] = x.y;
                kk[4 * u + 2] = x.z;
                kk[4 * u + 3] = x.w;
                ok |= in ? (0xFu << (4 * u)) : 0u;
            }
            scan_keys<K, false>(kk, ok, slo, shi, clt, ceqlo, ceqhi, st);
        }
    if (blockIdx.x == 0) {
        const bool okh = threadIdx.x < head, okt = threadIdx.x < n - tail0;
        const uint32_t kk[2] = {ord_word<F32>(okh ? p[threadIdx.x] : 0u),
                                ord_word<F32>(okt ? p[tail0 + threadIdx.x] : 0u)};
        scan_keys<2, false>(kk, (okh ? 1u : 0u) | (okt ? 2u : 0u), slo, shi, clt, ceqlo, ceqhi, st);
    }
    u64 r0 = clt, r1 = ceqlo, r2 = ceqhi;
#pragma unroll
    for (int o = WAVE / 2; o > 0; o >>= 1) {
        r0 += __shfl_xor(r0, o, WAVE);
        r1 += __shfl_xor(r1, o, WAVE);
        r2 += __shfl_xor(r2, o, WAVE);
    }
    if (lane == 0) {
        red[0][wid] = r0;
        red[1][wid] = r1;
        red[2][wid] = r2;
        red[3][wid] = (ORD ? os.winside : 0ull) + st.winside;
        red[4][wid] = st.wfill;
    }
    __syncthreads();
    if (threadIdx.x < 5) {
        u64 sum = 0;
        for (int w = 0; w < BLK / WAVE; ++w) sum += red[threadIdx.x][w];
        if (threadIdx.x == 4) {
            u64 g = 0;
            if (sum) {
                g = atomicAdd(a.cand_count, sum);
                if (g <= a.cap && g + sum > a.cap) atomicAdd(&a.stats_acc[C_OVF], 1ull);
            }
            red[5][0] = g;
        } else {
            const int slot[4] = {C_LT, C_EQLO, C_EQHI, C_IN};
            if (sum) atomicAdd(&a.stats_acc[slot[threadIdx.x]], sum);
        }
    }
    __syncthreads();
    bool grouped = false;
    if constexpr (TF == 0) {
        if (a.pre_hist) {
            __shared__ uint32_t phist[PRE_BINS];
            __shared__ uint32_t pflushed;
            const uint32_t W = cand_width(ss.lo, ss.hi);
            const uint32_t d = min(W, fin_first_digit(W)), sh = W - d, base = ss.lo + 1u;
            if (threadIdx.x == 0) pflushed = 0u;
            for (int b = threadIdx.x; b < PRE_BINS; b += BLK) phist[b] = 0u;
            __syncthreads();
            if (lane == 0 && st.flushed) atomicOr(&pflushed, 1u);
            __syncthreads();
            if (pflushed) {
                if (threadIdx.x == 0) atomicAdd(&a.pre_hist[PRE_INCOMPLETE], 1u);
            } else if (W > 0u) {
#pragma unroll
                for (int q = 0; q < BLK / WAVE; ++q) {
                    const uint32_t nq = (uint32_t)red[4][q];
                    for (uint32_t i = threadIdx.x; i < nq; i += BLK) {
                        const uint32_t b = (region[q][i] - base) >> sh, f = __builtin_amdgcn_readfirstlane(b);
                        const u64 act = __ballot(true);
                        if (__ballot(b != f) == 0) {
                            if ((uint32_t)lane == (uint32_t)__builtin_ctzll(act)) atomicAdd(&phist[f], (uint32_t)__popcll(act));
                        } else {
                            atomicAdd(&phist[b], 1u);
                        }
                    }
                }
                __syncthreads();
                uint32_t *dst = a.pre_hist + (blockIdx.x % PRE_COPIES) * PRE_BINS;
                for (uint32_t b = threadIdx.x; b < (1u << d); b += BLK) {
                    const uint32_t c = phist[b];
                    if (c) atomicAdd(&dst[b], c);
                }
                KTH_STAMP(a, 4);
                u64 tot = 0;
#pragma unroll
                for (int q = 0; q < BLK / WAVE; ++q) tot += red[4][q];
                const u64 g0 = red[5][0];
                if (tflags != nullptr && g0 + tot <= a.cap) {
                    grouped = true;
                    constexpr int PT = (BLK / WAVE) * WREG / BLK, PQ = WREG / BLK;
                    static_assert(WREG % BLK == 0 && PT <= 32, "a thread's keys of the flat regions, one validity bit each");
                    uint32_t *flat = &region[0][0];
                    uint32_t kk[PT], vm = 0;
#pragma unroll
                    for (int j = 0; j < PT; ++j) {
                        kk[j] = flat[j * BLK + threadIdx.x];
                        vm |= (uint32_t)((j % PQ) * BLK + threadIdx.x) < (uint32_t)red[4][j / PQ] ? 1u << j : 0u;
                    }
                    const uint32_t c0 = phist[4 * threadIdx.x], c1 = phist[4 * threadIdx.x + 1],
                                   c2 = phist[4 * threadIdx.x + 2], c3 = phist[4 * threadIdx.x + 3];
                    const uint32_t inc = wave_incl_scan32(c0 + c1 + c2 + c3);
                    if (lane == WAVE - 1) scratch[wid] = inc;
                    __syncthreads();
                    uint32_t e0 = inc - (c0 + c1 + c2 + c3);
                    for (int w = 0; w < wid; ++w) e0 += (uint32_t)scratch[w];
                    const uint32_t e1 = e0 + c0, e2 = e1 + c1, e3 = e2 + c2;
                    phist[4 * threadIdx.x] = e0;
                    phist[4 * threadIdx.x + 1] = e1;
                    phist[4 * threadIdx.x + 2] = e2;
                    phist[4 * threadIdx.x + 3] = e3;
                    u64 *row = reinterpret_cast<u64 *>(reinterpret_cast<uint8_t *>(tflags) + (size_t)blockIdx.x * GDIR_ROW_BYTES);
                    __hip_atomic_store(row + threadIdx.x, (u64)e0 | (u64)e1 << 16 | (u64)e2 << 32 | (u64)e3 << 48,
                                       __ATOMIC_RELAXED, __HIP_MEMORY_SCOPE_AGENT);
                    if (threadIdx.x == 0) {
                        __hip_atomic_store(row + PRE_BINS / 4, tot, __ATOMIC_RELAXED, __HIP_MEMORY_SCOPE_AGENT);
                        __hip_atomic_store(row + GDIR_BASE_OFF / 8, g0, __ATOMIC_RELAXED, __HIP_MEMORY_SCOPE_AGENT);
                    }
                    __syncthreads();
#pragma unroll
                    for (int j = 0; j < PT; ++j)
                        if ((vm >> j) & 1u) flat[atomicAdd(&phist[(kk[j] - base) >> sh], 1u)] = kk[j];
                    __syncthreads();
                    for (uint32_t i = threadIdx.x; i < (uint32_t)tot; i += BLK) put_cand(&cand_out[g0 + i], flat[i]);
                }
            }
        }
    }
    if (!grouped && st.wfill) {
        u64 g = red[5][0];
        for (int w = 0; w < wid; ++w) g += red[4][w];
        st.put(g, st.wfill);
    }
    KTH_STAMP(a, 5);
}

template <bool F32 = false>
__global__ __launch_bounds__(BLK) void k_result(StepArgs a, int32_t *d_out, int32_t *d_status, u64 *izero,
                                                u64 izero_words, uint32_t *last, uint32_t last_word) {
    __shared__ SelState ss;
    __shared__ u64 scratch[2 * (BLK / WAVE) + 8];
    KTH_STAMP(a, 0);
    advance<BLK>(ss, a, scratch);
    if (threadIdx.x == 0) {
        SelState o = ss;
        if (o.mode != MODE_DONE && !o.error) o.error = 16 + o.mode;
        *a.st_out = o;
        if (d_out && !o.error) *d_out = out_word<F32>(o.answer);
        if (d_status) {
            d_status[0] = i32_of_key(o.answer);
            d_status[1] = (int32_t)o.error;
        }
        if (last) *last = last_word;
    }
    __syncthreads();
    for (u64 i = threadIdx.x; i < izero_words; i += BLK) izero[i] = 0;
    KTH_STAMP(a, 5);
}

constexpr int DDIG = 12;
constexpr int DNB = 1 << DDIG;
static_assert(DNB == 2 * NBINS, "a stats slot's histogram words hold one DDIG-bit digit");
constexpr uint32_t DIST_FULL_D0 = 32 - 2 * DDIG;

struct CandDom {
    uint32_t base, W, d0;
};
__device__ __forceinline__ CandDom cand_domain(uint32_t lo, uint32_t hi) {
    CandDom d{lo + 1u, 0u, 0u};
    if (hi - lo < 2u) return d;
    const uint32_t range = hi - lo - 2u;
    d.W = range ? 32u - (uint32_t)__clz(range) : 0u;
// ... 381 lines not shown
```

mpi-k-selection_amd/kselect/__init__.py:

```python
import ctypes

import numpy as np

from ._lib import (
    KTH_DIST_DONE,
    KTH_DIST_MAX_LEVELS,
    KTH_ECOMM,
    KTH_EINTERNAL,
    KTH_EINVAL,
    KTH_ENODEV,
    KTH_FINISH_COUNTS,
    KTH_FINISH_GROUPED,
    KTH_FINISH_LEVELS,
    KTH_FINISH_NONE,
    KTH_FINISH_SLICES,
    KTH_HOOK_FAULT_BARRIER,
    KTH_HOOK_FAULT_TOPK_RANK,
    KTH_HOOK_FINISH_SLICES,
    KTH_HOOK_K16_MISS,
    KTH_HOOK_K16_TOPK_NOSKIP,
    KTH_HOOK_TOPK_SEG_CAP,
    KTH_MULTI_MAX_RANKS,
    KTH_K16_BF16,
    KTH_K16_F16,
# ... 223 lines not shown
            _need_f32(d_out, "d_out")
            check(LIB.kth_select_f32_async(self._ctx, _ptr(d_keys), int(n), int(k), _ptr(d_out)),
                  "kth_select_f32_async")
            return
        check(LIB.kth_select_i32_async(self._ctx, _ptr(d_keys), int(n), int(k), _ptr(d_out)),
              "kth_select_i32_async")

    def select_multi(self, keys, ks, n=None, f32=False):
        keys = _multi_host_keys(keys, f32)
        if n is None:
            n = _numel(keys)
        fn, what = ((LIB.kth_select_multi_f32_ctx, "kth_select_multi_f32_ctx") if f32
                    else (LIB.kth_select_multi_i32_ctx, "kth_select_multi_i32_ctx"))
        groups = list(_rank_groups(ks))
        out = np.empty(sum(len(g) for _, g in groups), dtype=np.float32 if f32 else np.int32)
        for at, g in groups:
            check(fn(self._ctx, _ptr(keys), int(n), g, len(g), out[at:].ctypes.data), what)
        return out

    def select_multi_async(self, d_keys, n, ks, d_out, f32=False):
        if f32:
            _need_f32(d_keys, "d_keys")
            _need_f32(d_out, "d_out")
        fn, what = ((LIB.kth_select_multi_f32_async, "kth_select_multi_f32_async") if f32
                    else (LIB.kth_select_multi_i32_async, "kth_select_multi_i32_async"))
        for at, g in _rank_groups(ks):
            check(fn(self._ctx, _ptr(d_keys), int(n), g, len(g), _ptr(d_out) + 4 * at), what)

    def reserve_multi(self, n, m):
        check(LIB.kth_ctx_reserve_multi(self._ctx, int(n), min(int(m), KTH_MULTI_MAX_RANKS)), "kth_ctx_reserve_multi")

    def multi_stats(self, i):
        st = KthStats()
        check(LIB.kth_ctx_multi_stats(self._ctx, int(i), ctypes.byref(st)), "kth_ctx_multi_stats")
        return st.as_dict()

    def select16(self, keys, k, n=None, kind=None):
        return self.select16_multi(keys, [k], n=n, kind=kind)[0]

    def select16_async(self, d_keys, n, k, d_out, kind=None):
        self.select16_multi_async(d_keys, n, [k], d_out, kind=kind)

    def select16_multi(self, keys, ks, n=None, kind=None):
        kind = _k16_kind(keys, kind)
        keys = _k16_host_keys(keys)
        if n is None:
            n = _numel(keys)
        groups = list(_rank_groups(ks))
        out = np.empty(sum(len(g) for _, g in groups), dtype=np.uint16)
        for at, g in groups:
            check(LIB.kth_select_multi_k16_ctx(self._ctx, _ptr(keys), int(n), g, len(g), kind, out[at:].ctypes.data),
                  "kth_select_multi_k16_ctx")
        return _k16_values(out, kind)

    def select16_multi_async(self, d_keys, n, ks, d_out, kind=None):
        kind = _k16_kind(d_keys, kind, "d_keys")
        _k16_kind(d_out, kind, "d_out")
        for at, g in _rank_groups(ks):
            check(LIB.kth_select_multi_k16_async(self._ctx, _ptr(d_keys), int(n), g, len(g), kind, _ptr(d_out) + 2 * at),
                  "kth_select_multi_k16_async")

    def reserve16(self, n, m=1):
        check(LIB.kth_ctx_reserve_k16(self._ctx, int(n), min(int(m), KTH_MULTI_MAX_RANKS)), "kth_ctx_reserve_k16")

    def coop(self):
        r = LIB.kth_ctx_coop(self._ctx)
        if r < 0:
            check(r, "kth_ctx_coop")
        return bool(r)

    def test_hook(self, hook, value):
        check(LIB.kth_ctx_test_hook(self._ctx, int(hook), int(value)), "kth_ctx_test_hook")

    def stats(self):
        st = KthStats()
        check(LIB.kth_ctx_last_stats(self._ctx, ctypes.byref(st)), "kth_ctx_last_stats")
        return st.as_dict()

    def finish_form(self):
        form = ctypes.c_int(-1)
        check(LIB.kth_ctx_last_finish_form(self._ctx, ctypes.byref(form)), "kth_ctx_last_finish_form")
        return form.value

    def rows(self, d_keys, rows, cols, k, d_out, f32=False):
        fn = LIB.kth_select_rows_f32 if f32 else LIB.kth_select_rows_i32
        check(fn(self._ctx, _ptr(d_keys), int(rows), int(cols), int(k), _ptr(d_out)), "kth_select_rows")

    def topk_rows(self, d_keys, rows, cols, k, d_vals=None, d_idx=None, largest=False, f32=False):
        fn = LIB.kth_topk_rows_f32 if f32 else LIB.kth_topk_rows_i32
        check(fn(self._ctx, _ptr(d_keys), int(rows), int(cols), int(k), 1 if largest else 0,
                 _ptr(d_vals) if d_vals is not None else None, _ptr(d_idx) if d_idx is not None else None),
              "kth_topk_rows")

    def rows16(self, d_keys, rows, cols, k, d_out, kind=None):
        kind = _k16_kind(d_keys, kind, "d_keys")
        _k16_same_kind(d_keys, d_out, kind, "d_out")
        check(LIB.kth_select_rows_k16(self._ctx, _ptr(d_keys), int(rows), int(cols), int(k), kind, _ptr(d_out)),
              "kth_select_rows_k16")

    def topk_rows16(self, d_keys, rows, cols, k, d_vals=None, d_idx=None, largest=False, kind=None):
        kind = _k16_kind(d_keys, kind, "d_keys")
        if d_vals is not None:
            _k16_same_kind(d_keys, d_vals, kind, "d_vals")
        dt = getattr(d_idx, "dtype", None)
        if dt is not None and str(dt).rsplit(".", 1)[-1] != "int32":
            raise TypeError(f"d_idx must be int32, got {dt}")
        check(LIB.kth_topk_rows_k16(self._ctx, _ptr(d_keys), int(rows), int(cols), int(k), 1 if largest else 0, kind,
                                    _ptr(d_vals) if d_vals is not None else None,
                                    _ptr(d_idx) if d_idx is not None else None), "kth_topk_rows_k16")

    def rows_wide(self, d_keys, rows, cols, k, d_out, f32=False, ld=None):
        if f32:
            _need_f32(d_keys, "d_keys")
            _need_f32(d_out, "d_out")
        fn, what = ((LIB.kth_select_wide_rows_f32, "kth_select_wide_rows_f32") if f32 else
                    (LIB.kth_select_wide_rows_i32, "kth_select_wide_rows_i32"))
        check(fn(self._ctx, _ptr(d_keys), int(rows), int(cols), int(cols if ld is None else ld), int(k), _ptr(d_out)),
              what)

    def topk_rows_wide(self, d_keys, rows, cols, k, d_vals=None, d_idx=None, largest=False, f32=False, ld=None):
        if f32:
            _need_f32(d_keys, "d_keys")
            _need_f32(d_vals, "d_vals")
        dt = getattr(d_idx, "dtype", None)
        if dt is not None and str(dt).rsplit(".", 1)[-1] != "int32":
            raise TypeError(f"d_idx must be int32, got {dt}")
        fn, what = ((LIB.kth_topk_wide_rows_f32, "kth_topk_wide_rows_f32") if f32 else
                    (LIB.kth_topk_wide_rows_i32, "kth_topk_wide_rows_i32"))
        check(fn(self._ctx, _ptr(d_keys), int(rows), int(cols), int(cols if ld is None else ld), int(k),
                 1 if largest else 0, _ptr(d_vals) if d_vals is not None else None,
                 _ptr(d_idx) if d_idx is not None else None), what)

    def rows_wide16(self, d_keys, rows, cols, k, d_out, kind=None, ld=None):
        kind = _k16_kind(d_keys, kind, "d_keys")
        _k16_same_kind(d_keys, d_out, kind, "d_out")
        check(LIB.kth_select_wide_rows_k16(self._ctx, _ptr(d_keys), int(rows), int(cols),
                                           int(cols if ld is None else ld), int(k), kind, _ptr(d_out)),
              "kth_select_wide_rows_k16")

    def topk_rows_wide16(self, d_keys, rows, cols, k, d_vals=None, d_idx=None, largest=False, kind=None, ld=None):
        kind = _k16_kind(d_keys, kind, "d_keys")
        if d_vals is not None:
            _k16_same_kind(d_keys, d_vals, kind, "d_vals")
        dt = getattr(d_idx, "dtype", None)
        if dt is not None and str(dt).rsplit(".", 1)[-1] != "int32":
            raise TypeError(f"d_idx must be int32, got {dt}")
        check(LIB.kth_topk_wide_rows_k16(self._ctx, _ptr(d_keys), int(rows), int(cols), int(cols if ld is None else ld),
                                         int(k), 1 if largest else 0, kind,
                                         _ptr(d_vals) if d_vals is not None else None,
                                         _ptr(d_idx) if d_idx is not None else None), "kth_topk_wide_rows_k16")

    def rows_wide_var(self, d_keys, rows, cols, k, d_out, f32=False, d_lens=None, d_ks=None, ld=None):
        if f32:
            _need_f32(d_keys, "d_keys")
            _need_f32(d_out, "d_out")
        _need_i32(d_lens, "d_lens")
        _need_i32(d_ks, "d_ks")
        fn, what = ((LIB.kth_select_wide_rows_var_f32, "kth_select_wide_rows_var_f32") if f32 else
                    (LIB.kth_select_wide_rows_var_i32, "kth_select_wide_rows_var_i32"))
        check(fn(self._ctx, _ptr(d_keys), int(rows), int(cols), int(cols if ld is None else ld), _ptr_or_none(d_lens),
                 _ptr_or_none(d_ks), int(k), _ptr(d_out)), what)

    def topk_rows_wide_var(self, d_keys, rows, cols, k, d_vals=None, d_idx=None, largest=False, f32=False,
                           d_lens=None, d_ks=None, d_cnt=None, ld=None):
        if f32:
            _need_f32(d_keys, "d_keys")
# ... 322 lines not shown
```

mpi-k-selection_amd/kselect/_lib.py:

```python
import ctypes
import os

HERE = os.path.dirname(os.path.abspath(__file__))
PKG_ROOT = os.path.dirname(HERE)
LIB_PATH = os.environ.get("KTH_LIB") or os.path.join(PKG_ROOT, "lib", "libkth.so")

KTH_OK = 0
KTH_EINVAL = -1
KTH_ENOMEM = -2
KTH_EHIP = -3
KTH_ENODEV = -4
KTH_EINTERNAL = -5
KTH_ECOMM = -6

KTH_PATH_LDS, KTH_PATH_RADIX, KTH_PATH_WINDOW, KTH_PATH_WINDOW_FALLBACK = 1, 2, 3, 4
KTH_PATH_K16, KTH_PATH_K16_FALLBACK = 5, 6
KTH_K16_I16, KTH_K16_U16, KTH_K16_F16, KTH_K16_BF16 = 0, 1, 2, 3
KTH_STATS_WORDS = 8 + 2 * 2048
KTH_DIST_DONE = 3
KTH_DIST_MAX_LEVELS = 3
KTH_ROWS_MAX_COLS = 16384
KTH_TOPK_MAX_COLS = 4096
KTH_ROWS16_MAX_COLS = 8192
KTH_WIDE_MAX_COLS = 1 << 24
# ... 9 lines not shown
c_u32p = ctypes.POINTER(ctypes.c_uint32)
c_u64p = ctypes.POINTER(ctypes.c_uint64)
c_i64p = ctypes.POINTER(ctypes.c_int64)
c_vp = ctypes.c_void_p


class KthStats(ctypes.Structure):
    _fields_ = [
        ("path", ctypes.c_int32),
        ("mode", ctypes.c_int32),
        ("lo_key", ctypes.c_uint32),
        ("hi_key", ctypes.c_uint32),
        ("n", ctypes.c_uint64),
        ("k", ctypes.c_uint64),
        ("cnt_lt", ctypes.c_uint64),
        ("cnt_eq_lo", ctypes.c_uint64),
        ("cnt_eq_hi", ctypes.c_uint64),
        ("candidates", ctypes.c_uint64),
        ("capacity", ctypes.c_uint64),
        ("answer", ctypes.c_int32),
        ("error", ctypes.c_int32),
    ]

    def as_dict(self):
        return {f: getattr(self, f) for f, _ in self._fields_}


class IntVector(ctypes.Structure):
    _fields_ = [("size", ctypes.c_int), ("capacity", ctypes.c_int), ("data", ctypes.POINTER(ctypes.c_int))]


IntVectorPtr = ctypes.POINTER(IntVector)


class KthError(RuntimeError):
    def __init__(self, code, what=""):
        self.code = code
        super().__init__(f"{what}: {code} ({strerror(code)})" if what else f"{code} ({strerror(code)})")


class KthLibraryMissing(ImportError):
    pass


PROTOS = {
    "kth_strerror": (ctypes.c_char_p, [ctypes.c_int]),
    "kth_version": (ctypes.c_int, []),
    "kth_build_id": (ctypes.c_char_p, []),
    "kth_device_count": (ctypes.c_int, []),
    "kth_select_i32": (ctypes.c_int, [c_vp, ctypes.c_int64, ctypes.c_int64, c_i32p]),
    "kth_ctx_create": (ctypes.c_int, [ctypes.c_int, ctypes.POINTER(c_vp)]),
    "kth_ctx_destroy": (ctypes.c_int, [c_vp]),
    "kth_ctx_set_stream": (ctypes.c_int, [c_vp, c_vp]),
    "kth_ctx_sync": (ctypes.c_int, [c_vp]),
    "kth_ctx_reserve": (ctypes.c_int, [c_vp, ctypes.c_int64]),
    "kth_select_i32_ctx": (ctypes.c_int, [c_vp, c_vp, ctypes.c_int64, ctypes.c_int64, c_i32p]),
    "kth_select_i32_async": (ctypes.c_int, [c_vp, c_vp, ctypes.c_int64, ctypes.c_int64, c_vp]),
    "kth_select_f32": (ctypes.c_int, [c_vp, ctypes.c_int64, ctypes.c_int64, c_vp]),
    "kth_select_f32_ctx": (ctypes.c_int, [c_vp, c_vp, ctypes.c_int64, ctypes.c_int64, c_vp]),
    "kth_select_f32_async": (ctypes.c_int, [c_vp, c_vp, ctypes.c_int64, ctypes.c_int64, c_vp]),
    "kth_select_multi_i32": (ctypes.c_int, [c_vp, ctypes.c_int64, c_i64p, ctypes.c_int, c_vp]),
    "kth_select_multi_i32_ctx": (ctypes.c_int, [c_vp, c_vp, ctypes.c_int64, c_i64p, ctypes.c_int, c_vp]),
    "kth_select_multi_i32_async": (ctypes.c_int, [c_vp, c_vp, ctypes.c_int64, c_i64p, ctypes.c_int, c_vp]),
    "kth_select_multi_f32": (ctypes.c_int, [c_vp, ctypes.c_int64, c_i64p, ctypes.c_int, c_vp]),
    "kth_select_multi_f32_ctx": (ctypes.c_int, [c_vp, c_vp, ctypes.c_int64, c_i64p, ctypes.c_int, c_vp]),
    "kth_select_multi_f32_async": (ctypes.c_int, [c_vp, c_vp, ctypes.c_int64, c_i64p, ctypes.c_int, c_vp]),
    "kth_ctx_reserve_multi": (ctypes.c_int, [c_vp, ctypes.c_int64, ctypes.c_int]),
    "kth_ctx_multi_stats": (ctypes.c_int, [c_vp, ctypes.c_int, ctypes.POINTER(KthStats)]),
    "kth_k16_order_key": (ctypes.c_uint16, [ctypes.c_uint16, ctypes.c_int]),
    "kth_k16_of_order_key": (ctypes.c_uint16, [ctypes.c_uint16, ctypes.c_int]),
    "kth_select_k16": (ctypes.c_int, [c_vp, ctypes.c_int64, ctypes.c_int64, ctypes.c_int, c_vp]),
    "kth_select_k16_ctx": (ctypes.c_int, [c_vp, c_vp, ctypes.c_int64, ctypes.c_int64, ctypes.c_int, c_vp]),
    "kth_select_k16_async": (ctypes.c_int, [c_vp, c_vp, ctypes.c_int64, ctypes.c_int64, ctypes.c_int, c_vp]),
    "kth_select_multi_k16": (ctypes.c_int, [c_vp, ctypes.c_int64, c_i64p, ctypes.c_int, ctypes.c_int, c_vp]),
    "kth_select_multi_k16_ctx": (ctypes.c_int, [c_vp, c_vp, ctypes.c_int64, c_i64p, ctypes.c_int, ctypes.c_int, c_vp]),
    "kth_select_multi_k16_async": (ctypes.c_int, [c_vp, c_vp, ctypes.c_int64, c_i64p, ctypes.c_int, ctypes.c_int, c_vp]),
    "kth_ctx_reserve_k16": (ctypes.c_int, [c_vp, ctypes.c_int64, ctypes.c_int]),
    "kth_f32_order_key": (ctypes.c_uint32, [ctypes.c_float]),
    "kth_f32_of_order_key": (ctypes.c_float, [ctypes.c_uint32]),
    "kth_ctx_last_stats": (ctypes.c_int, [c_vp, ctypes.POINTER(KthStats)]),
    "kth_ctx_coop": (ctypes.c_int, [c_vp]),
    "kth_ctx_test_hook": (ctypes.c_int, [c_vp, ctypes.c_int, ctypes.c_int64]),
    "kth_ctx_last_finish_form": (ctypes.c_int, [c_vp, ctypes.POINTER(ctypes.c_int)]),
    "kth_ctx_enable_timing": (ctypes.c_int, [c_vp, ctypes.c_int]),
    "kth_ctx_take_timing": (ctypes.c_int, [c_vp, ctypes.POINTER(ctypes.c_int64), ctypes.POINTER(ctypes.c_double),
                                           ctypes.POINTER(ctypes.c_double)]),
    "kth_select_rows_i32": (ctypes.c_int, [c_vp, c_vp, ctypes.c_int64, ctypes.c_int32, ctypes.c_int32, c_vp]),
    "kth_select_rows_f32": (ctypes.c_int, [c_vp, c_vp, ctypes.c_int64, ctypes.c_int32, ctypes.c_int32, c_vp]),
    "kth_topk_rows_i32": (ctypes.c_int, [c_vp, c_vp, ctypes.c_int64, ctypes.c_int32, ctypes.c_int32, ctypes.c_int,
                                         c_vp, c_vp]),
    "kth_topk_rows_f32": (ctypes.c_int, [c_vp, c_vp, ctypes.c_int64, ctypes.c_int32, ctypes.c_int32, ctypes.c_int,
                                         c_vp, c_vp]),
    "kth_select_rows_k16": (ctypes.c_int, [c_vp, c_vp, ctypes.c_int64, ctypes.c_int32, ctypes.c_int32, ctypes.c_int,
                                           c_vp]),
    "kth_topk_rows_k16": (ctypes.c_int, [c_vp, c_vp, ctypes.c_int64, ctypes.c_int32, ctypes.c_int32, ctypes.c_int,
                                         ctypes.c_int, c_vp, c_vp]),
    "kth_select_wide_rows_i32": (ctypes.c_int, [c_vp, c_vp, ctypes.c_int64, ctypes.c_int32, ctypes.c_int64,
                                                ctypes.c_int32, c_vp]),
    "kth_select_wide_rows_f32": (ctypes.c_int, [c_vp, c_vp, ctypes.c_int64, ctypes.c_int32, ctypes.c_int64,
                                                ctypes.c_int32, c_vp]),
    "kth_topk_wide_rows_i32": (ctypes.c_int, [c_vp, c_vp, ctypes.c_int64, ctypes.c_int32, ctypes.c_int64, ctypes.c_int32,
                                              ctypes.c_int, c_vp, c_vp]),
    "kth_topk_wide_rows_f32": (ctypes.c_int, [c_vp, c_vp, ctypes.c_int64, ctypes.c_int32, ctypes.c_int64, ctypes.c_int32,
                                              ctypes.c_int, c_vp, c_vp]),
    "kth_ctx_reserve_wide_rows": (ctypes.c_int, [c_vp, ctypes.c_int64, ctypes.c_int32]),
    "kth_wide_rows_plan": (ctypes.c_int, [ctypes.c_int64, ctypes.c_int32, ctypes.c_int, c_i32p, c_i32p, c_i32p, c_i64p]),
    "kth_ctx_wide_rows_force": (ctypes.c_int, [c_vp, ctypes.c_int32, ctypes.c_int32]),
    "kth_select_wide_rows_k16": (ctypes.c_int, [c_vp, c_vp, ctypes.c_int64, ctypes.c_int32, ctypes.c_int64,
                                                ctypes.c_int32, ctypes.c_int, c_vp]),
    "kth_topk_wide_rows_k16": (ctypes.c_int, [c_vp, c_vp, ctypes.c_int64, ctypes.c_int32, ctypes.c_int64, ctypes.c_int32,
                                              ctypes.c_int, ctypes.c_int, c_vp, c_vp]),
    "kth_wide_rows_plan_k16": (ctypes.c_int, [ctypes.c_int64, ctypes.c_int32, ctypes.c_int, c_i32p, c_i32p, c_i32p,
                                              c_i64p]),
    "kth_select_wide_rows_var_i32": (ctypes.c_int, [c_vp, c_vp, ctypes.c_int64, ctypes.c_int32, ctypes.c_int64, c_vp,
                                                    c_vp, ctypes.c_int32, c_vp]),
    "kth_select_wide_rows_var_f32": (ctypes.c_int, [c_vp, c_vp, ctypes.c_int64, ctypes.c_int32, ctypes.c_int64, c_vp,
                                                    c_vp, ctypes.c_int32, c_vp]),
    "kth_select_wide_rows_var_k16": (ctypes.c_int, [c_vp, c_vp, ctypes.c_int64, ctypes.c_int32, ctypes.c_int64, c_vp,
                                                    c_vp, ctypes.c_int32, ctypes.c_int, c_vp]),
    "kth_topk_wide_rows_var_i32": (ctypes.c_int, [c_vp, c_vp, ctypes.c_int64, ctypes.c_int32, ctypes.c_int64, c_vp, c_vp,
                                                  ctypes.c_int32, ctypes.c_int, c_vp, c_vp, c_vp]),
    "kth_topk_wide_rows_var_f32": (ctypes.c_int, [c_vp, c_vp, ctypes.c_int64, ctypes.c_int32, ctypes.c_int64, c_vp, c_vp,
                                                  ctypes.c_int32, ctypes.c_int, c_vp, c_vp, c_vp]),
    "kth_topk_wide_rows_var_k16": (ctypes.c_int, [c_vp, c_vp, ctypes.c_int64, ctypes.c_int32, ctypes.c_int64, c_vp, c_vp,
                                                  ctypes.c_int32, ctypes.c_int, ctypes.c_int, c_vp, c_vp, c_vp]),
    "kth_nucleus_wide_rows_f32": (ctypes.c_int, [c_vp, c_vp, ctypes.c_int64, ctypes.c_int32, ctypes.c_int64, c_vp, c_vp,
                                                 ctypes.c_float, c_vp, ctypes.c_float, c_vp, c_vp]),
    "kth_nucleus_wide_rows_k16": (ctypes.c_int, [c_vp, c_vp, ctypes.c_int64, ctypes.c_int32, ctypes.c_int64, c_vp, c_vp,
                                                 ctypes.c_float, c_vp, ctypes.c_float, ctypes.c_int, c_vp, c_vp]),
    "kth_topp_wide_rows_f32": (ctypes.c_int, [c_vp, c_vp, ctypes.c_int64, ctypes.c_int32, ctypes.c_int64, c_vp, c_vp,
                                              ctypes.c_int32, c_vp, ctypes.c_float, c_vp, ctypes.c_float, c_vp, c_vp,
                                              c_vp]),
    "kth_topp_wide_rows_k16": (ctypes.c_int, [c_vp, c_vp, ctypes.c_int64, ctypes.c_int32, ctypes.c_int64, c_vp, c_vp,
                                              ctypes.c_int32, c_vp, ctypes.c_float, c_vp, ctypes.c_float, ctypes.c_int,
                                              c_vp, c_vp, c_vp]),
    "kth_ctx_reserve_topp_rows": (ctypes.c_int, [c_vp, ctypes.c_int64, ctypes.c_int32]),
    "kth_sample_wide_rows_f32": (ctypes.c_int, [c_vp, c_vp, ctypes.c_int64, ctypes.c_int32, ctypes.c_int64, c_vp, c_vp,
                                                ctypes.c_int32, c_vp, ctypes.c_float, c_vp, ctypes.c_float, c_vp, c_vp,
                                                c_vp]),
    "kth_sample_wide_rows_k16": (ctypes.c_int, [c_vp, c_vp, ctypes.c_int64, ctypes.c_int32, ctypes.c_int64, c_vp, c_vp,
                                                ctypes.c_int32, c_vp, ctypes.c_float, c_vp, ctypes.c_float, c_vp,
                                                ctypes.c_int, c_vp, c_vp]),
    "kth_ctx_reserve_sample_rows": (ctypes.c_int, [c_vp, ctypes.c_int64, ctypes.c_int32]),
    "kth_topk_i32": (ctypes.c_int, [c_vp, c_vp, ctypes.c_int64, ctypes.c_int64, ctypes.c_int, c_vp, c_vp]),
    "kth_topk_f32": (ctypes.c_int, [c_vp, c_vp, ctypes.c_int64, ctypes.c_int64, ctypes.c_int, c_vp, c_vp]),
    "kth_topk_k16": (ctypes.c_int, [c_vp, c_vp, ctypes.c_int64, ctypes.c_int64, ctypes.c_int, ctypes.c_int, c_vp, c_vp]),
    "kth_ctx_last_topk_k16_tiles": (ctypes.c_int, [c_vp, c_u64p, c_u64p]),
    "kth_fill_synthetic": (ctypes.c_int, [c_vp, c_vp, ctypes.c_int64, ctypes.c_int64, ctypes.c_int64, ctypes.c_int,
                                          ctypes.c_uint64, ctypes.c_int32]),
    "kth_dist_begin": (ctypes.c_int, [c_vp, c_vp, ctypes.c_int64, ctypes.c_int64]),
    "kth_dist_sample": (ctypes.c_int, [c_vp, c_vp, ctypes.c_int64, c_vp, ctypes.c_int64]),
    "kth_dist_window": (ctypes.c_int, [c_vp, c_vp, ctypes.c_int64]),
    "kth_dist_scan": (ctypes.c_int, [c_vp, c_vp, ctypes.c_int64]),
    "kth_dist_level": (ctypes.c_int, [c_vp, c_vp, ctypes.c_int64, ctypes.c_int]),
    "kth_dist_result": (ctypes.c_int, [c_vp, c_vp]),
    "kth_dist_result_early": (ctypes.c_int, [c_vp, c_vp]),
    "kth_dist_select_rccl": (ctypes.c_int, [c_vp, c_vp, c_vp, c_vp, ctypes.c_int, c_vp, ctypes.c_int64, ctypes.c_int64,
                                            ctypes.c_int64, c_vp, c_vp, c_vp, ctypes.c_int64, c_vp, ctypes.c_int]),
    "kth_dist_sample_size": (ctypes.c_int64, [ctypes.c_int64]),
    "kth_sample_chunk": (ctypes.c_int, []),
    "kth_window_z": (ctypes.c_double, []),
    "kth_dist_cand_capacity": (ctypes.c_int64, [ctypes.c_int64]),
    "kth_window_slack64": (ctypes.c_int, []),
    "kth_sharded_create": (ctypes.c_int, [c_vp, ctypes.c_int, ctypes.POINTER(c_vp)]),
    "kth_sharded_destroy": (ctypes.c_int, [c_vp]),
    "kth_sharded_select_i32": (ctypes.c_int, [c_vp, c_vp, c_vp, ctypes.c_int64, c_i32p]),
# ... 82 lines not shown
```

Baseline: 1613 Gkeys/s.

## Decide finish bin inside main kernel and pass resident key rows to finisher

Measured after the change: 1629 Gkeys/s, median of 6. No clear change (+1.0%).

```diff
diff --git a/include/kth.h b/include/kth.h
--- a/include/kth.h
+++ b/include/kth.h
@@ -98,6 +98,8 @@
 #define KTH_FINISH_GROUPED 3
 #define KTH_FINISH_LEVELS 4
 int kth_ctx_last_finish_form(kth_ctx *ctx, int *form);
+
+int kth_ctx_last_resident_rows(kth_ctx *ctx, int *rows);
 
 int kth_ctx_coop(const kth_ctx *ctx);
 
diff --git a/mpi-k-selection_amd/csrc/kth_api.hip b/mpi-k-selection_amd/csrc/kth_api.hip
--- a/mpi-k-selection_amd/csrc/kth_api.hip
+++ b/mpi-k-selection_amd/csrc/kth_api.hip
@@ -52,7 +52,11 @@
 constexpr size_t ZERO_WORDS = PRE_OFF + (size_t)kth::PRE_WORDS / 2;
 constexpr size_t BAR_OFF = ZERO_WORDS;
 constexpr size_t TAIL_OFF = BAR_OFF + kth::BAR_WORDS / 2;
-constexpr size_t SLOT_ALLOC_WORDS = TAIL_OFF + kth::FIN_LDS_KEYS / 2;
+constexpr size_t ROWS_OFF = TAIL_OFF + kth::FIN_LDS_KEYS / 2;
+constexpr size_t COPIES_OFF = ROWS_OFF + (size_t)kth::RES_ROWS_MAX * kth::RES_ROW_WORDS / 2;
+constexpr size_t SLOT_ALLOC_WORDS = COPIES_OFF + (size_t)kth::RES_SHARDS * kth::RES_SHARD_STRIDE / 2;
+static_assert((COPIES_OFF - BAR_OFF) * 2 == (size_t)kth::RES_COPIES, "the kernels find the copies from the barrier state");
+static_assert((ROWS_OFF - BAR_OFF) * 2 == (size_t)kth::RES_TABLE, "the kernels find the table from the barrier state");
 static_assert(kth::BAR_TAIL % 2 == 0, "the tail word is a u64");
 constexpr u64 FIN_SPARSE_PER_WG = (u64)kth::DENSE_BLK * kth::FIN_UNROLL * 4;
 constexpr double HEAD_SLACK = 1.5;
@@ -139,6 +143,7 @@
     uint32_t head_abs_div = 1024;
     bool pre_hist = true;
     bool group = true;
+    bool resident = true;
     bool finish_slices = false;
     hipStream_t stream = nullptr;
     bool own_stream = false;
@@ -483,15 +488,15 @@
 
 template <bool F32>
 void launch_finish(kth_ctx *c, const StepArgs &a, int32_t *d_out, int32_t *d_status, uint32_t last, bool with_pre = false,
-                   u64 *head_slots = nullptr, int group_rows = 0) {
+                   u64 *head_slots = nullptr, int group_rows = 0, bool resident = false) {
     kth::CoopArgs x = coop_args(c, FSLOT_OFF, d_out, d_status);
     x.zero2 = head_slots ? head_slots : c->islots + HSLOT_OFF;
     x.zero2_words = HSLOT_WORDS;
     x.pre = with_pre ? pre_words(c) : nullptr;
     x.last = d_last(c);
-    kth::FinGroup fg{nullptr, 0u};
+    kth::FinGroup fg{nullptr, 0u, 0u};
     if (with_pre && group_rows > 0 && !c->finish_slices)
-        fg = kth::FinGroup{reinterpret_cast<const uint8_t *>(c->gdir.p), (uint32_t)group_rows};
+        fg = kth::FinGroup{reinterpret_cast<const uint8_t *>(c->gdir.p), (uint32_t)group_rows, resident ? 1u : 0u};
     kth::k_finish<F32><<<c->fin_grid, kth::DENSE_BLK, FIN_DYN_LDS, c->stream>>>(a, x, last, fg);
 }
 
@@ -534,7 +539,8 @@
 }
 
 template <bool F32>
-void launch_main(kth_ctx *c, const StepArgs &a, int tflag, uint32_t *tflags, uint32_t *gdir = nullptr) {
+void launch_main(kth_ctx *c, const StepArgs &a, int tflag, uint32_t *tflags, uint32_t *gdir = nullptr,
+                 uint32_t *res_bar = nullptr) {
     const kth::TkSeg none{};
     if (F32 && tflag >= 5) tflag = 0;
     const int g = c->main_grid[F32][tflag];
@@ -550,7 +556,7 @@
     case 6:
         if constexpr (!F32) kth::k_main<6><<<g, kth::BLK, 0, c->stream>>>(a, cand, tflags, nullptr, c->tk_seg);
         break;
-    default: kth::k_main<0, F32><<<g, kth::BLK, 0, c->stream>>>(a, cand, gdir, nullptr, none); break;
+    default: kth::k_main<0, F32><<<g, kth::BLK, 0, c->stream>>>(a, cand, gdir, res_bar, none); break;
     }
 }
 
@@ -566,6 +572,10 @@
 
     if (c->coop) {
         Chain ch{c, c->islots, 2};
+        const bool pre = tflag == 0 && c->pre_hist;
+        const bool grp = pre && grouping(c) && c->gdir.p != nullptr;
+        const bool res = grp && c->resident && !c->finish_slices && !c->fault_barrier && c->main_wg_per_cu == 0 &&
+                         c->main_grid[F32][0] <= kth::RES_ROWS_MAX;
         StepArgs a = head_step(ch, n, k, s, r_lo, r_hi, true);
         kth::CoopArgs hx = coop_args(c, HSLOT_OFF, nullptr, nullptr);
         if (tflag == 0 && c->head_abs_div) hx.abs_min = (u64)s / c->head_abs_div;
@@ -573,15 +583,14 @@
                                                                                c->sample.p, (u64)s);
         a = ch.next(kth::ADV_CARRY, Chain::ACC);
         over_keys(a, keys, n);
-        const bool pre = tflag == 0 && c->pre_hist;
         if (pre) a.pre_hist = pre_words(c);
-        const bool grp = pre && grouping(c) && c->gdir.p != nullptr;
         ev_main(c);
-        launch_main<F32>(c, a, tflag, tflags, grp ? c->gdir.p : nullptr);
+        launch_main<F32>(c, a, tflag, tflags, grp ? c->gdir.p : nullptr,
+                         res ? reinterpret_cast<uint32_t *>(c->islots + BAR_OFF) : nullptr);
         ev_main(c);
         a = ch.next(kth::ADV_DECIDE, Chain::IN);
         over_keys(a, keys, n);
-        launch_finish<F32>(c, a, d_out, d_status, single_word<F32>(c, 0), pre, nullptr, grp ? c->main_grid[F32][0] : 0);
+        launch_finish<F32>(c, a, d_out, d_status, single_word<F32>(c, 0), pre, nullptr, grp ? c->main_grid[F32][0] : 0, res);
         c->last_state = 0;
         c->counts_left = true;
         return launch_check();
@@ -1186,6 +1195,7 @@
     if (const char *g = getenv("KTH_COOP")) c->coop = atoi(g) != 0;
     if (const char *g = getenv("KTH_PRE_HIST")) c->pre_hist = atoi(g) != 0;
     if (const char *g = getenv("KTH_GROUP")) c->group = atoi(g) != 0;
+    if (const char *g = getenv("KTH_RESIDENT")) c->resident = atoi(g) != 0;
     c->fin_grid = c->num_cu;
     if (const char *g = getenv("KTH_FIN_GRID")) c->fin_grid = std::max(1, std::min(atoi(g), c->num_cu));
     if (const char *g = getenv("KTH_HEAD_SLACK")) c->head_slack64 = (uint32_t)std::max(0.0, atof(g) * 64.0);
@@ -2033,6 +2043,16 @@
     KTH_TRY(fetch_last(c, &last));
     if (last.form == LAST_NONE) return KTH_EINVAL;
     *form = (int)((uint32_t)c->h_status[2] >> kth::LAST_FORM_SHIFT & 7u);
+    if (*form == (int)kth::FORM_ROWS) *form = KTH_FINISH_GROUPED;
+    return KTH_OK;
+}
+
+int kth_ctx_last_resident_rows(kth_ctx *c, int *rows) {
+    if (!c || !rows) return KTH_EINVAL;
+    LastCall last;
+    KTH_TRY(fetch_last(c, &last));
+    if (last.form == LAST_NONE) return KTH_EINVAL;
+    *rows = ((uint32_t)c->h_status[2] >> kth::LAST_FORM_SHIFT & 7u) == kth::FORM_ROWS ? 1 : 0;
     return KTH_OK;
 }
 
diff --git a/mpi-k-selection_amd/csrc/kth_coop.hpp b/mpi-k-selection_amd/csrc/kth_coop.hpp
--- a/mpi-k-selection_amd/csrc/kth_coop.hpp
+++ b/mpi-k-selection_amd/csrc/kth_coop.hpp
@@ -164,6 +164,7 @@
 constexpr int FIN_LDS_KEYS = 32768;
 constexpr int FIN_UNROLL = 4;
 constexpr uint32_t LAST_FORM_SHIFT = 12;
+constexpr uint32_t FORM_ROWS = 5;
 
 __device__ __forceinline__ void finish_keys(uint32_t (*lh)[NBINS], const HistPlan &plan, const uint4 &x, bool xr,
                                             uint32_t valid4) {
@@ -403,8 +404,41 @@
 struct FinGroup {
     const uint8_t *dir;
     uint32_t rows;
+    uint32_t resident;
 };
 constexpr int GATHER_UNROLL = 8;
+static_assert(RES_MAX_KEYS == (uint32_t)FIN_LDS_KEYS, "a bin picked for resident rows fits the finisher's LDS");
+static_assert(RES_ROWS_MAX <= DENSE_BLK, "one thread of k_finish reads each row");
+
+template <bool SKIP>
+__device__ __forceinline__ void gather_keys(const StepArgs &a, const uint32_t *off, const u64 *src, uint32_t tot,
+                                            uint32_t *rw, uint32_t pad) {
+    for (uint32_t i0 = 0; i0 < tot; i0 += GATHER_UNROLL * DENSE_BLK) {
+        uint32_t v[GATHER_UNROLL];
+        bool have[GATHER_UNROLL];
+#pragma unroll
+        for (int u = 0; u < GATHER_UNROLL; ++u) {
+            const uint32_t i = i0 + u * DENSE_BLK + threadIdx.x;
+            v[u] = pad;
+            have[u] = i < tot;
+            if (i < tot) {
+                uint32_t s = 0;
+#pragma unroll
+                for (uint32_t step = DENSE_BLK / 2; step; step >>= 1) s += off[s + step] <= i ? step : 0u;
+                const u64 at = src[s] + (i - off[s]);
+                if (SKIP && src[s] == ~0ull)
+                    have[u] = false;
+                else if (at < a.cap)
+                    v[u] = load_nt(a.cand + at);
+            }
+        }
+#pragma unroll
+        for (int u = 0; u < GATHER_UNROLL; ++u) {
+            const uint32_t i = i0 + u * DENSE_BLK + threadIdx.x;
+            if (have[u]) rw[i] = v[u];
+        }
+    }
+}
 template <bool F32>
 __device__ bool finish_gather(const StepArgs &a, SelState &ss, const FinGroup &fg, uint4 *res, u64 cnt0,
                               uint32_t (*lh)[NBINS], u64 *scratch, uint32_t *total_out) {
@@ -436,26 +470,61 @@
     }
     const uint32_t tot = (uint32_t)total;
     uint32_t *rw = reinterpret_cast<uint32_t *>(res);
-    for (uint32_t i0 = 0; i0 < tot; i0 += GATHER_UNROLL * DENSE_BLK) {
-        uint32_t v[GATHER_UNROLL];
-#pragma unroll
-        for (int u = 0; u < GATHER_UNROLL; ++u) {
-            const uint32_t i = i0 + u * DENSE_BLK + threadIdx.x;
-            v[u] = pad;
-            if (i < tot) {
-                uint32_t s = 0;
-#pragma unroll
-                for (uint32_t step = DENSE_BLK / 2; step; step >>= 1) s += off[s + step] <= i ? step : 0u;
-                const u64 at = src[s] + (i - off[s]);
-                if (at < a.cap) v[u] = load_nt(a.cand + at);
-            }
-        }
-#pragma unroll
-        for (int u = 0; u < GATHER_UNROLL; ++u) {
-            const uint32_t i = i0 + u * DENSE_BLK + threadIdx.x;
-            if (i < tot) rw[i] = v[u];
-        }
-    }
+    gather_keys<false>(a, off, src, tot, rw, pad);
+    if (threadIdx.x < 3 && tot + threadIdx.x < ((tot + 3) & ~3u)) rw[tot + threadIdx.x] = pad;
+    __syncthreads();
+    KTH_STAMP(a, 6);
+    *total_out = tot;
+    return true;
+}
+
+template <bool F32>
+__device__ bool finish_rows(const StepArgs &a, SelState &ss, const uint32_t *tab, uint32_t rows, uint4 *res, u64 cnt0,
+                            uint32_t (*lh)[NBINS], u64 *scratch, uint32_t *total_out) {
+    __shared__ uint32_t s_far;
+    uint32_t *off = &lh[0][0];
+    u64 *src = reinterpret_cast<u64 *>(&lh[1][0]);
+    const uint32_t pad = finisher_pad(ss);
+    uint32_t w[RES_ROW_WORDS];
+#pragma unroll
+    for (int j = 0; j < RES_ROW_WORDS; ++j) w[j] = 0u;
+    if (threadIdx.x < rows) {
+#pragma unroll
+        for (int j = 0; j <= RES_ROW_FIRST; ++j) w[j] = load_nt(tab + (size_t)j * RES_ROWS_MAX + threadIdx.x);
+    }
+    if (threadIdx.x == 0) s_far = 0u;
+    const bool far = (w[0] & RES_ROW_FAR) != 0u;
+    uint32_t cnt = w[0] & ~RES_ROW_FAR;
+    if (!far && cnt > (uint32_t)RES_ROW_INLINE) cnt = ~0u;
+    if (__syncthreads_or(!far && cnt != ~0u && cnt > (uint32_t)RES_ROW_FIRST)) {
+        if (threadIdx.x < rows && !far && cnt != ~0u && cnt > (uint32_t)RES_ROW_FIRST) {
+#pragma unroll
+            for (int j = RES_ROW_FIRST + 1; j < RES_ROW_WORDS; ++j) w[j] = load_nt(tab + (size_t)j * RES_ROWS_MAX + threadIdx.x);
+        }
+    }
+    u64 total;
+    const uint32_t at = (uint32_t)block_exclusive_scan<DENSE_BLK>((u64)cnt, scratch, &total);
+    off[threadIdx.x] = at;
+    src[threadIdx.x] = far ? ((u64)w[2] << 32 | w[1]) : ~0ull;
+    if (far && cnt) s_far = 1u;
+    __syncthreads();
+    KTH_STAMP(a, 5);
+    if (total != cnt0 || total > (u64)FIN_LDS_KEYS) {
+        if (threadIdx.x == 0) {
+            ss.error = 34;
+            ss.mode = MODE_DONE;
+        }
+        __syncthreads();
+        return false;
+    }
+    const uint32_t tot = (uint32_t)total;
+    uint32_t *rw = reinterpret_cast<uint32_t *>(res);
+    if (!far) {
+#pragma unroll
+        for (int j = 0; j < RES_ROW_INLINE; ++j)
+            if ((uint32_t)j < cnt) rw[at + j] = w[j + 1];
+    }
+    if (s_far) gather_keys<true>(a, off, src, tot, rw, pad);
     if (threadIdx.x < 3 && tot + threadIdx.x < ((tot + 3) & ~3u)) rw[tot + threadIdx.x] = pad;
     __syncthreads();
     KTH_STAMP(a, 6);
@@ -476,12 +545,21 @@
     GridBar gb = grid_bar_init(x.bar, s_base);
     for (int i = threadIdx.x; i < 2 * NBINS / 4; i += DENSE_BLK) reinterpret_cast<uint4 *>(&lh[0][0])[i] = make_uint4(0, 0, 0, 0);
     const uint32_t pre_incomplete = x.pre ? x.pre[PRE_INCOMPLETE] : 1u;
+    u64 rec_dec = 0, rec_cnt = 0, rec_below = 0;
+    if (fg.resident) {
+        const u64 *rec = reinterpret_cast<const u64 *>(x.bar + BAR_RES);
+        rec_dec = rec[0];
+        rec_cnt = rec[RES_COUNT / 2];
+        rec_below = rec[RES_BELOW / 2];
+    }
     [[clang::always_inline]] advance<DENSE_BLK>(ss, a, scratch);
     if (threadIdx.x == 0 && (ss.mode == MODE_CAND || ss.mode == MODE_FULL) && ss.t[0].done == 0)
         ss.d0 = fin_first_digit(ss.W);
     __syncthreads();
     const bool use_pre = pre_incomplete == 0u && ss.mode == MODE_CAND && ss.t[0].done == 0;
     const bool group = use_pre && fg.dir != nullptr && fg.rows <= (uint32_t)DENSE_BLK && !x.fault;
+    const uint32_t rdec = (uint32_t)(rec_dec >> 32);
+    const bool rows = group && (rdec & 0xFFu) == RES_PICK;
     KTH_STAMP(a, 1);
     const uint32_t mode0 = ss.mode;
     const bool live = mode0 == MODE_CAND || mode0 == MODE_FULL;
@@ -511,6 +589,26 @@
         }
         const bool pre0 = L == 0 && use_pre;
         const uint32_t nb = plan.mask[0] + 1u, copies = L == 0 ? NBINS / nb : 1u;
+        if (pre0 && rows) {
+            if (threadIdx.x == 0) {
+                const uint32_t d = digit_bits(ss, 0u), bin = rdec >> 8, cnt = (uint32_t)rec_cnt;
+                const u64 kk = ss.t[0].k;
+                if (d >= ss.W || bin >= (1u << d) || cnt == 0u || cnt > (uint32_t)FIN_LDS_KEYS || rec_below >= kk ||
+                    kk - rec_below > (u64)cnt) {
+                    ss.error = 34;
+                    ss.mode = MODE_DONE;
+                } else {
+                    ss.t[0].k = kk - rec_below;
+                    ss.t[0].prefix = bin;
+                    ss.t[0].done = d;
+                }
+                s_cnt0 = cnt;
+            }
+            __syncthreads();
+            gather = true;
+            KTH_STAMP(a, 4);
+            break;
+        }
         if (pre0 && group) {
             pick_pre<DENSE_BLK>(ss, x.pre, nb, scratch, &s_cnt0, &s_ptot);
             if (s_ptot != ss.cnt[C_IN] ||
@@ -630,15 +728,23 @@
     }
     if (levels > 0 && !tail && !gather) grid_sync(gb, s_base, ok);
     grid_bar_finish(gb, s_base);
+    if (fg.resident && blockIdx.x == 0) {
+        if (threadIdx.x < BAR_NG) x.bar[BAR_CENSUS + threadIdx.x * RES_CENSUS_STRIDE] = 0u;
+        if (threadIdx.x < RES_BELOW + 2) x.bar[BAR_RES + threadIdx.x] = 0u;
+        if (threadIdx.x < RES_SHARDS) x.bar[RES_COPIES + threadIdx.x * RES_SHARD_STRIDE] = 0u;
+    }
     bool writer = blockIdx.x == 0, finisher = false;
     uint32_t fin_keys = 0;
     if (tail) {
         [[clang::always_inline]] writer = finisher = finish_tail<F32>(a, ss, x, res, nk, xr, lh, scratch, &fin_keys);
     } else if (gather && (ss.mode == MODE_CAND || ss.mode == MODE_FULL)) {
-        [[clang::always_inline]] finisher = finish_gather<F32>(a, ss, fg, res, s_cnt0, lh, scratch, &fin_keys);
+        if (rows)
+            [[clang::always_inline]] finisher = finish_rows<F32>(a, ss, x.bar + RES_TABLE, fg.rows, res, s_cnt0, lh, scratch, &fin_keys);
+        else
+            [[clang::always_inline]] finisher = finish_gather<F32>(a, ss, fg, res, s_cnt0, lh, scratch, &fin_keys);
     }
     if (finisher && !ss.error) finish_levels<F32>(a, ss, res, fin_keys, lh, scratch);
-    const uint32_t form = levels == 0 ? 1u : tail ? 2u : gather ? 3u : 4u;
+    const uint32_t form = levels == 0 ? 1u : tail ? 2u : gather ? (rows ? FORM_ROWS : 3u) : 4u;
     if (writer && threadIdx.x == 0) {
         SelState o = ss;
         const uint32_t berr = __hip_atomic_exchange(x.bar + BAR_ERR, 0u, __ATOMIC_RELAXED, __HIP_MEMORY_SCOPE_AGENT);
diff --git a/mpi-k-selection_amd/csrc/kth_gridbar.hpp b/mpi-k-selection_amd/csrc/kth_gridbar.hpp
--- a/mpi-k-selection_amd/csrc/kth_gridbar.hpp
+++ b/mpi-k-selection_amd/csrc/kth_gridbar.hpp
@@ -13,9 +13,21 @@
 constexpr int BAR_TAIL = BAR_ERR + BAR_GROUP_STRIDE;
 constexpr int BAR_TAIL_WRITTEN = BAR_TAIL + 32;
 constexpr int BAR_TOPK_ARRIVE = BAR_TAIL + 48;
-constexpr int BAR_WORDS = BAR_TAIL + BAR_GROUP_STRIDE;
-static_assert(BAR_TAIL_WRITTEN >= BAR_TAIL + 2 && BAR_TOPK_ARRIVE > BAR_TAIL_WRITTEN && BAR_TOPK_ARRIVE < BAR_WORDS,
+constexpr int BAR_RES = BAR_TAIL + BAR_GROUP_STRIDE;
+constexpr int RES_DECISION = 1, RES_COUNT = 2, RES_BELOW = 4;
+constexpr int RES_CENSUS_STRIDE = 32;
+constexpr int BAR_CENSUS = BAR_RES + BAR_GROUP_STRIDE;
+constexpr int BAR_WORDS = BAR_CENSUS + BAR_NG * RES_CENSUS_STRIDE;
+static_assert(BAR_TAIL_WRITTEN >= BAR_TAIL + 2 && BAR_TOPK_ARRIVE > BAR_TAIL_WRITTEN && BAR_TOPK_ARRIVE < BAR_RES,
               "the tail word (u64), its written count and the top-k arrival counter are distinct words");
+static_assert(BAR_RES % 2 == 0 && RES_BELOW % 2 == 0 && BAR_WORDS % 2 == 0, "the resident-rows line holds u64 words");
+constexpr uint32_t RES_EMPTY = 0u, RES_PICK = 1u, RES_SPILL = 2u, RES_ABORT = 3u;
+constexpr int RES_ROW_WORDS = 32, RES_ROW_INLINE = RES_ROW_WORDS - 1, RES_ROWS_MAX = 1024;
+constexpr int RES_ROW_FIRST = 16;
+constexpr int RES_SHARDS = 128, RES_SHARD_STRIDE = 1088;
+constexpr uint32_t RES_ROW_FAR = 0x80000000u;
+constexpr uint32_t RES_MAX_KEYS = 32768;
+constexpr u64 RES_CENSUS_TICKS = 20000;
 static_assert(BAR_NG <= WAVE && BAR_NG <= BAR_GROUP_STRIDE, "one wave polls every group; the bases fit one stride");
 constexpr uint32_t BAR_SPIN_LIMIT = 1u << 21;
 constexpr uint32_t ERR_BARRIER = 64;
diff --git a/mpi-k-selection_amd/csrc/kth_kernels.hip b/mpi-k-selection_amd/csrc/kth_kernels.hip
--- a/mpi-k-selection_amd/csrc/kth_kernels.hip
+++ b/mpi-k-selection_amd/csrc/kth_kernels.hip
@@ -897,6 +897,114 @@
 }
 static_assert(MAIN_UNROLL <= 8, "k_main<TF> keeps one row bit per 16-B load slot in a byte");
 static_assert(BLK / WAVE == 4, "k_main<TF> stores one flag byte per wave, four per tile (tk_row_flagged's mask)");
+constexpr int RES_TABLE = BAR_WORDS + (int)RES_MAX_KEYS;
+constexpr int RES_COPIES = RES_TABLE + RES_ROWS_MAX * RES_ROW_WORDS;
+
+__device__ __forceinline__ void resident_publish(uint32_t *bar, uint32_t dec, uint32_t first, uint32_t step) {
+    for (uint32_t i = first; i < (uint32_t)RES_SHARDS; i += step)
+        __hip_atomic_store(bar + RES_COPIES + i * RES_SHARD_STRIDE, dec, __ATOMIC_RELAXED, __HIP_MEMORY_SCOPE_AGENT);
+}
+
+__device__ __forceinline__ void resident_decide(SelState &ss, const StepArgs &a, uint32_t *bar, u64 *scratch,
+                                                uint32_t sh, uint32_t *s_dec) {
+    __shared__ uint32_t s_bin, s_cnt;
+    __shared__ u64 s_below;
+    const int lane = threadIdx.x & (WAVE - 1), wid = threadIdx.x / WAVE;
+    if (threadIdx.x < 5)
+        scratch[threadIdx.x] = __hip_atomic_load(a.stats_acc + threadIdx.x, __ATOMIC_RELAXED, __HIP_MEMORY_SCOPE_AGENT);
+    if (threadIdx.x == 5)
+        scratch[5] = __hip_atomic_load(a.pre_hist + PRE_INCOMPLETE, __ATOMIC_RELAXED, __HIP_MEMORY_SCOPE_AGENT);
+    if (threadIdx.x == 6) s_bin = ~0u;
+    const CoherentBuf pb(a.pre_hist, PRE_COPIES * PRE_BINS * 4);
+    uint32_t c0 = 0, c1 = 0, c2 = 0, c3 = 0;
+#pragma unroll
+    for (int q = 0; q < PRE_COPIES; ++q) {
+        const uint4 v = pb.load16((uint32_t)(q * PRE_BINS + 4 * threadIdx.x) * 4u);
+        c0 += v.x;
+        c1 += v.y;
+        c2 += v.z;
+        c3 += v.w;
+    }
+    __syncthreads();
+    if (threadIdx.x == 0) decide(ss, scratch);
+    __syncthreads();
+    const bool cand = ss.mode == MODE_CAND && scratch[5] == 0 && sh > 0u;
+    const uint32_t sum = c0 + c1 + c2 + c3, inc = wave_incl_scan32(sum);
+    if (lane == WAVE - 1) scratch[8 + wid] = inc;
+    __syncthreads();
+    uint32_t ex = inc - sum, total = 0;
+#pragma unroll
+    for (int w = 0; w < BLK / WAVE; ++w) {
+        if (w < wid) ex += (uint32_t)scratch[8 + w];
+        total += (uint32_t)scratch[8 + w];
+    }
+    const u64 kk = ss.t[0].k;
+    if (cand && (u64)ex < kk && kk <= (u64)ex + sum) {
+        uint32_t b = 0, below = ex, cnt = c0;
+        if (kk > (u64)below + cnt) below += cnt, cnt = c1, b = 1;
+        if (b == 1 && kk > (u64)below + cnt) below += cnt, cnt = c2, b = 2;
+        if (b == 2 && kk > (u64)below + cnt) below += cnt, cnt = c3, b = 3;
+        s_bin = 4 * threadIdx.x + b;
+        s_cnt = cnt;
+        s_below = below;
+    }
+    __syncthreads();
+    if (threadIdx.x == 0) {
+        uint32_t want = RES_SPILL;
+        if (cand && s_bin != ~0u && (u64)total == ss.cnt[C_IN] && s_cnt <= RES_MAX_KEYS) {
+            __hip_atomic_store(bar + BAR_RES + RES_COUNT, s_cnt, __ATOMIC_RELAXED, __HIP_MEMORY_SCOPE_AGENT);
+            __hip_atomic_store(reinterpret_cast<u64 *>(bar + BAR_RES + RES_BELOW), s_below, __ATOMIC_RELAXED,
+                               __HIP_MEMORY_SCOPE_AGENT);
+            wait_mem();
+            want = RES_PICK | s_bin << 8;
+        }
+        uint32_t seen = RES_EMPTY;
+        const bool won = __hip_atomic_compare_exchange_strong(bar + BAR_RES + RES_DECISION, &seen, want, __ATOMIC_RELAXED,
+                                                              __ATOMIC_RELAXED, __HIP_MEMORY_SCOPE_AGENT);
+        *s_dec = won ? want : seen;
+        s_cnt = won ? 1u : 0u;
+    }
+    __syncthreads();
+    if (s_cnt) resident_publish(bar, *s_dec, threadIdx.x, BLK);
+}
+
+__device__ __forceinline__ uint32_t resident_wait(uint32_t *bar) {
+    const uint32_t lane = threadIdx.x & (WAVE - 1);
+    const uint32_t groups = gridDim.x < (uint32_t)BAR_NG ? gridDim.x : (uint32_t)BAR_NG;
+    const uint32_t *mine = bar + RES_COPIES + (blockIdx.x % RES_SHARDS) * RES_SHARD_STRIDE;
+    const u64 t0 = __builtin_amdgcn_s_memrealtime();
+    bool started = false;
+    uint32_t spins = 0, dec;
+    while (true) {
+        dec = (uint32_t)__builtin_amdgcn_readfirstlane(
+            (int)__hip_atomic_load(mine, __ATOMIC_RELAXED, __HIP_MEMORY_SCOPE_AGENT));
+        if (dec != RES_EMPTY) break;
+        bool give_up = ++spins >= BAR_SPIN_LIMIT;
+        if (!started) {
+            uint32_t s = lane < groups ? __hip_atomic_load(bar + BAR_CENSUS + lane * RES_CENSUS_STRIDE, __ATOMIC_RELAXED,
+                                                           __HIP_MEMORY_SCOPE_AGENT)
+                                       : 0u;
+#pragma unroll
+            for (int o = WAVE / 2; o > 0; o >>= 1) s += __shfl_xor(s, o, WAVE);
+            started = s == gridDim.x;
+            give_up = give_up || (!started && __builtin_amdgcn_s_memrealtime() - t0 > RES_CENSUS_TICKS);
+        }
+        if (give_up) {
+            uint32_t seen = RES_EMPTY;
+            if (lane == 0 &&
+                __hip_atomic_compare_exchange_strong(bar + BAR_RES + RES_DECISION, &seen, RES_ABORT, __ATOMIC_RELAXED,
+                                                     __ATOMIC_RELAXED, __HIP_MEMORY_SCOPE_AGENT))
+                seen = RES_EMPTY | 0x100u;
+            seen = (uint32_t)__builtin_amdgcn_readfirstlane((int)seen);
+            dec = seen == (RES_EMPTY | 0x100u) ? RES_ABORT : seen;
+            if (seen == (RES_EMPTY | 0x100u)) resident_publish(bar, RES_ABORT, lane, WAVE);
+            break;
+        }
+        __builtin_amdgcn_s_sleep(24);
+    }
+    return dec;
+}
+
 template <int TF, bool F32 = false>
 __global__ __launch_bounds__(BLK) void k_main(StepArgs a, uint32_t *__restrict__ cand_out,
                                               uint32_t *__restrict__ tflags, uint32_t *__restrict__ cand_rows,
@@ -932,6 +1040,11 @@
     if (ss.mode != MODE_MAIN) return;
     const int32_t slo = i32_of_key(ss.lo), shi = i32_of_key(ss.hi);
     const int lane = threadIdx.x & (WAVE - 1), wid = threadIdx.x / WAVE;
+    if constexpr (TF == 0) {
+        if (cand_rows != nullptr && threadIdx.x == 0)
+            __hip_atomic_fetch_add(cand_rows + BAR_CENSUS + (blockIdx.x % BAR_NG) * RES_CENSUS_STRIDE, 1u, __ATOMIC_RELAXED,
+                                   __HIP_MEMORY_SCOPE_AGENT);
+    }
     if constexpr (TF != 0) {
         if (blockIdx.x == 0 && threadIdx.x == 0) {
             tflags[0] = (uint32_t)slo;
@@ -1172,9 +1285,11 @@
             __syncthreads();
             if (lane == 0 && st.flushed) atomicOr(&pflushed, 1u);
             __syncthreads();
+            bool counted = false;
             if (pflushed) {
                 if (threadIdx.x == 0) atomicAdd(&a.pre_hist[PRE_INCOMPLETE], 1u);
             } else if (W > 0u) {
+                counted = true;
 #pragma unroll
                 for (int q = 0; q < BLK / WAVE; ++q) {
                     const uint32_t nq = (uint32_t)red[4][q];
@@ -1194,12 +1309,73 @@
                     const uint32_t c = phist[b];
                     if (c) atomicAdd(&dst[b], c);
                 }
-                KTH_STAMP(a, 4);
-                u64 tot = 0;
-#pragma unroll
-                for (int q = 0; q < BLK / WAVE; ++q) tot += red[4][q];
-                const u64 g0 = red[5][0];
-                if (tflags != nullptr && g0 + tot <= a.cap) {
+            }
+            KTH_STAMP(a, 4);
+            u64 tot = 0;
+#pragma unroll
+            for (int q = 0; q < BLK / WAVE; ++q) tot += red[4][q];
+            const u64 g0 = red[5][0];
+            const bool can_group = counted && tflags != nullptr && g0 + tot <= a.cap;
+            uint32_t dec = RES_SPILL;
+            if (cand_rows != nullptr) {
+                __shared__ uint32_t s_last, s_dec;
+                wait_mem();
+                __syncthreads();
+                if (threadIdx.x == 0)
+                    s_last = __hip_atomic_fetch_add(cand_rows + BAR_RES, 1u, __ATOMIC_RELAXED, __HIP_MEMORY_SCOPE_AGENT) ==
+                             gridDim.x - 1u;
+                KTH_STAMP(a, 2);
+                __syncthreads();
+                if (s_last) {
+                    resident_decide(ss, a, cand_rows, scratch, sh, &s_dec);
+                } else {
+                    if (wid == 0) {
+                        const uint32_t got = resident_wait(cand_rows);
+                        if (lane == 0) s_dec = got;
+                    }
+                    __syncthreads();
+                }
+                dec = s_dec;
+                KTH_STAMP(a, 3);
+            }
+            if (can_group && (dec & 0xFFu) == RES_PICK) {
+                __shared__ uint32_t s_rowk[RES_ROW_INLINE];
+                grouped = true;
+                const uint32_t pb = dec >> 8, c = pb < (uint32_t)PRE_BINS ? phist[pb] : 0u;
+                const bool far = c > (uint32_t)RES_ROW_INLINE;
+                __syncthreads();
+                if (threadIdx.x == 0) phist[0] = 0u;
+                __syncthreads();
+#pragma unroll
+                for (int q = 0; q < BLK / WAVE; ++q) {
+                    const uint32_t nq = (uint32_t)red[4][q];
+                    for (uint32_t i = threadIdx.x; i < nq; i += BLK) {
+                        const uint32_t key = region[q][i];
+                        if (((key - base) >> sh) == pb) {
+                            const uint32_t at = atomicAdd(&phist[0], 1u);
+                            if (far) {
+                                if ((u64)at < tot) put_cand(&cand_out[g0 + at], key);
+                            } else if (at < (uint32_t)RES_ROW_INLINE) {
+                                s_rowk[at] = key;
+                            }
+                        }
+                    }
+                }
+                __syncthreads();
+                if (threadIdx.x < (uint32_t)RES_ROW_WORDS) {
+                    const uint32_t t = threadIdx.x;
+                    uint32_t word;
+                    if (t == 0)
+                        word = far ? c | RES_ROW_FAR : c;
+                    else if (far)
+                        word = t == 1 ? (uint32_t)g0 : t == 2 ? (uint32_t)(g0 >> 32) : 0u;
+                    else
+                        word = t - 1u < c ? s_rowk[t - 1u] : 0u;
+                    if (t <= (far ? 2u : c)) put_cand(cand_rows + RES_TABLE + (size_t)t * RES_ROWS_MAX + blockIdx.x, word);
+                }
+                wait_mem();
+            } else if (can_group) {
+                {
                     grouped = true;
                     constexpr int PT = (BLK / WAVE) * WREG / BLK, PQ = WREG / BLK;
                     static_assert(WREG % BLK == 0 && PT <= 32, "a thread's keys of the flat regions, one validity bit each");
diff --git a/mpi-k-selection_amd/kselect/__init__.py b/mpi-k-selection_amd/kselect/__init__.py
--- a/mpi-k-selection_amd/kselect/__init__.py
+++ b/mpi-k-selection_amd/kselect/__init__.py
@@ -329,6 +329,11 @@
         check(LIB.kth_ctx_last_finish_form(self._ctx, ctypes.byref(form)), "kth_ctx_last_finish_form")
         return form.value
 
+    def resident_rows(self):
+        rows = ctypes.c_int(-1)
+        check(LIB.kth_ctx_last_resident_rows(self._ctx, ctypes.byref(rows)), "kth_ctx_last_resident_rows")
+        return rows.value == 1
+
     def rows(self, d_keys, rows, cols, k, d_out, f32=False):
         fn = LIB.kth_select_rows_f32 if f32 else LIB.kth_select_rows_i32
         check(fn(self._ctx, _ptr(d_keys), int(rows), int(cols), int(k), _ptr(d_out)), "kth_select_rows")
diff --git a/mpi-k-selection_amd/kselect/_lib.py b/mpi-k-selection_amd/kselect/_lib.py
--- a/mpi-k-selection_amd/kselect/_lib.py
+++ b/mpi-k-selection_amd/kselect/_lib.py
@@ -115,6 +115,7 @@
     "kth_ctx_coop": (ctypes.c_int, [c_vp]),
     "kth_ctx_test_hook": (ctypes.c_int, [c_vp, ctypes.c_int, ctypes.c_int64]),
     "kth_ctx_last_finish_form": (ctypes.c_int, [c_vp, ctypes.POINTER(ctypes.c_int)]),
+    "kth_ctx_last_resident_rows": (ctypes.c_int, [c_vp, ctypes.POINTER(ctypes.c_int)]),
     "kth_ctx_enable_timing": (ctypes.c_int, [c_vp, ctypes.c_int]),
     "kth_ctx_take_timing": (ctypes.c_int, [c_vp, ctypes.POINTER(ctypes.c_int64), ctypes.POINTER(ctypes.c_double),
                                            ctypes.POINTER(ctypes.c_double)]),
```
